# victorramirez952/tomography_3d_reconstructor

Hardware: NVIDIA B200
Metric: Gvoxels/s mask-stack->mesh+volume (higher is better)
Workload: dtype u8 -> bit-packed u32 (topology), f64 field taps -> f32 vertices

## Files before the change

tomography_3d_reconstructor_b200/csrc/t3d_common.cuh:

```cuda
#pragma once
#include <cuda_runtime.h>
#include <stdint.h>
#include <stdio.h>

int t3d_num_sms(void);
#define T3D_NUM_SMS (t3d_num_sms())
bool t3d_first_use_on_device(int slot);
enum { T3D_ONCE_FILL_HOLES_ATTR = 0, T3D_ONCE_MC_LUTS = 1, T3D_ONCE_SORT_ATTR = 2, T3D_ONCE_MORPH4_ATTR = 3, T3D_ONCE_SLOTS = 8 };

extern "C" void t3d_set_error(const char* fmt, ...);
extern "C" void t3d_count_launches(int n);
int t3d_zero_async(void* p, size_t n, cudaStream_t st);
void t3d_prezero_register(const void* p, size_t n);
void t3d_prezero_clear(void);
void t3d_canonicalize_structured_zero_range(int64_t V, int64_t F, uint32_t cap_z, uint32_t cap_g0, int Zs, int64_t* offset,
                                            int64_t* size);

#define T3D_CHECK_LAUNCH(name)                                                                   \
    do {                                                                                         \
        cudaError_t e__ = cudaGetLastError();                                                    \
        if (e__ != cudaSuccess) {                                                                \
            t3d_set_error("%s: launch failed: %s", name, cudaGetErrorString(e__));               \
            return 1;                                                                            \
        }                                                                                        \
    } while (0)

#define T3D_CUDA(call)                                                                           \
    do {                                                                                         \
        cudaError_t e__ = (call);                                                                \
        if (e__ != cudaSuccess) {                                                                \
            t3d_set_error("%s failed: %s", #call, cudaGetErrorString(e__));                      \
            return 1;                                                                            \
        }                                                                                        \
    } while (0)

static inline int t3d_wpr(int W) { return (((W + 31) >> 5) + 3) & ~3; }
static inline int t3d_wvalid(int W) { return (W + 31) >> 5; }

__device__ __forceinline__ uint32_t lane_id() { return threadIdx.x & 31; }

__device__ __forceinline__ uint32_t valid_mask(int w, int W)
{
    const int rem = W - (w << 5);
    if (rem >= 32) return 0xffffffffu;
    if (rem <= 0) return 0u;
    return (1u << rem) - 1u;
}

template <typename T>
__device__ __forceinline__ T warp_sum(T v)
{
#pragma unroll
    for (int o = 16; o > 0; o >>= 1) v += __shfl_xor_sync(0xffffffffu, v, o);
    return v;
}

__device__ __forceinline__ int warp_min(int v)
{
#pragma unroll
    for (int o = 16; o > 0; o >>= 1) v = min(v, __shfl_xor_sync(0xffffffffu, v, o));
    return v;
}
__device__ __forceinline__ int warp_max(int v)
{
#pragma unroll
    for (int o = 16; o > 0; o >>= 1) v = max(v, __shfl_xor_sync(0xffffffffu, v, o));
    return v;
}

__device__ __forceinline__ uint32_t warp_incl_scan(uint32_t v)
{
    const uint32_t l = lane_id();
#pragma unroll
    for (int o = 1; o < 32; o <<= 1) {
        uint32_t t = __shfl_up_sync(0xffffffffu, v, o);
        if (l >= (uint32_t)o) v += t;
    }
    return v;
}

__device__ __forceinline__ uint4 ld_stream_u4(const void* p)
{
    uint4 r;
    asm volatile("ld.global.nc.L1::no_allocate.v4.u32 {%0,%1,%2,%3}, [%4];"
                 : "=r"(r.x), "=r"(r.y), "=r"(r.z), "=r"(r.w)
                 : "l"(p));
    return r;
}
__device__ __forceinline__ void st_stream_u4(void* p, uint4 v)
{
    asm volatile("st.global.L1::no_allocate.v4.u32 [%0], {%1,%2,%3,%4};" ::"l"(p), "r"(v.x), "r"(v.y),
                 "r"(v.z), "r"(v.w)
                 : "memory");
}

__device__ __forceinline__ uint32_t ge4(uint32_t v, uint32_t thr4)
{
    const uint32_t m = __vcmpgeu4(v, thr4) & 0x80808080u;
    return (m * 0x00204081u) >> 28;
}
__device__ __forceinline__ uint32_t ge16(uint4 v, uint32_t thr4)
{
    return ge4(v.x, thr4) | (ge4(v.y, thr4) << 4) | (ge4(v.z, thr4) << 8) | (ge4(v.w, thr4) << 12);
}
__device__ __forceinline__ uint32_t expand4(uint32_t nib) { return (nib * 0x00204081u) & 0x01010101u; }

__device__ __forceinline__ uint4 and4(uint4 a, uint4 b) { return make_uint4(a.x & b.x, a.y & b.y, a.z & b.z, a.w & b.w); }
__device__ __forceinline__ uint4 or4(uint4 a, uint4 b) { return make_uint4(a.x | b.x, a.y | b.y, a.z | b.z, a.w | b.w); }
__device__ __forceinline__ uint4 splat4(uint32_t v) { return make_uint4(v, v, v, v); }
__device__ __forceinline__ uint32_t popc4(uint4 a) { return __popc(a.x) + __popc(a.y) + __popc(a.z) + __popc(a.w); }
__device__ __forceinline__ uint4 valid_mask4(int w4, int W)
{
    return make_uint4(valid_mask(4 * w4, W), valid_mask(4 * w4 + 1, W), valid_mask(4 * w4 + 2, W), valid_mask(4 * w4 + 3, W));
}
__device__ __forceinline__ uint4 shl1_4(uint4 c, uint32_t l)
{
    return make_uint4(__funnelshift_l(l, c.x, 1), __funnelshift_l(c.x, c.y, 1), __funnelshift_l(c.y, c.z, 1), __funnelshift_l(c.z, c.w, 1));
}
__device__ __forceinline__ uint4 shr1_4(uint4 c, uint32_t r)
{
    return make_uint4(__funnelshift_r(c.x, c.y, 1), __funnelshift_r(c.y, c.z, 1), __funnelshift_r(c.z, c.w, 1), __funnelshift_r(c.w, r, 1));
}

__device__ __forceinline__ int64_t dev_n(int64_t cap, const unsigned long long* p)
{
    if (!p) return cap;
    const unsigned long long v = *p;
    return v < (unsigned long long)cap ? (int64_t)v : cap;
}

int t3d_morph_stage(const uint32_t* in, uint32_t* out, int Z, int H, int W, int z0, int nz, int out_rs, long long out_ps,
                    bool erode, bool ring, int ring_tail, unsigned long long* counts, cudaStream_t st);
bool t3d_morph4_eligible(int Z, int H, int W);
int t3d_morph4_launch(const uint32_t* in, uint32_t* out, int Z, int H, int W, int z0, int nz, int out_rs, long long out_ps, int ring_tail,
                      unsigned long long* counts, cudaStream_t st);
void t3d_canon_faces_ready_event(cudaEvent_t e);
bool t3d_canon_faces_ready_pending();
bool t3d_pack_gap_supported(const void* masks_u8, int Z, int H, int W, int threshold);
int t3d_pack_gap_launch(const void* masks_u8, int Z, int H, int W, int threshold, void* out, unsigned long long* counts,
                        unsigned int* bbox_t, int skip_ends, cudaStream_t st, int z_bias = 0);
int t3d_bbox_t_planes_launch(const uint32_t* bits, int n_planes, int H, int W, int z_bias, unsigned int* bbox_t, cudaStream_t st);
int t3d_close_ends_fixup_launch(const void* masks_u8, int Z, int H, int W, int threshold, const void* filled0, const void* filledT,
                                void* out, unsigned long long* counts, cudaStream_t st);
```

tomography_3d_reconstructor_b200/csrc/t3d_pipeline.cu:

```cuda
#include <stdint.h>

#include <stdlib.h>

#include <nvtx3/nvToolsExt.h>

#include "t3d.h"
#include "t3d_field.cuh"

struct NvtxRange {
    bool open;
    explicit NvtxRange(const char* name) : open(true) { nvtxRangePushA(name); }
    void end() { if (open) { nvtxRangePop(); open = false; } }
    ~NvtxRange() { end(); }
};

enum {
    R_NACTIVE = 0, R_NX = 1, R_NY = 2, R_NZ = 3, R_NT = 4, R_VCANON = 5, R_FCANON = 6, R_UNVERIFIED = 7, R_OVERFLOW = 8,
    R_NAMBIGUOUS = 9, R_NEXACT = 10, R_VOLUME_F64 = 11, R_AREA_F64 = 12, R_BBOX_I32X6 = 13 , R_VRAW = 16, R_NEXC = 17,
    R_NGHOST = 18, R_NLEAD = 19, R_NG0 = 25,
    R_COUNTS = 32
};

#define EXC_CAP (1u << 20)
#define SURF_HALO 3

#define S_XPAD 128

static inline int64_t al(int64_t x) { return (x + 255) & ~(int64_t)255; }

static bool fast_surface(int n_stages, unsigned erode_mask, int pad, int Zx, int H, int W)
{
    return pad == 1 && n_stages == 4 && (erode_mask & 15u) == 9u && Zx >= 2 && H >= 2 && W >= 2;
}

struct Layout {
    int64_t bitsA, bitsB, bitsC, morph, fill, sign, exc, ballots, chunkbase, scan1, aw_idx, aw_cnt, aw_base, scan2, vkeys, verts_raw,
        faces_raw, canon, measure, total;
};

static Layout make_layout(int Zx, int Zl, int H, int W, int pad, uint32_t capNA, uint32_t capV, uint32_t capF, uint32_t capZ,
                          uint32_t capG0, int n_stages, bool own_bitsA, bool fast)
{
    Layout L;
    const int64_t nw = t3d_words_per_row(W), vol = (int64_t)Zx * H * nw * 4;
    const int Zp = Zl + 2 * pad, Hp = H + 2 * pad, Wp = fast ? W + S_XPAD + 1 : W + 2 * pad;
    const int64_t nwp = t3d_words_per_row(Wp), n_chunks = t3d_mc_num_chunks(Zp, Hp, Wp);
    int64_t o = 0;
    L.bitsA = o; o += own_bitsA ? al(vol) : 0;
    L.bitsB = o; o += al(vol);
    L.bitsC = o; o += fast ? 0 : al(vol);
    L.morph = o; o += al(t3d_morph_scratch_bytes(Zx, H, W, n_stages));
    L.fill = o; o += al(t3d_fill_holes_scratch_bytes(2, H, W));
    L.sign = o; o += al((int64_t)Zp * Hp * nwp * 4);
    L.exc = o; o += al((int64_t)EXC_CAP * 8);
    L.ballots = o; o += al(n_chunks * 4);
    L.chunkbase = o; o += al(n_chunks * 4);
    L.scan1 = o; o += al(t3d_scan_workspace_bytes(n_chunks, 1));
    L.aw_idx = o; o += al((int64_t)capNA * 4);
    L.aw_cnt = o; o += al((int64_t)capNA * 16);
    L.aw_base = o; o += al((int64_t)capNA * 16);
    L.scan2 = o; o += al(t3d_scan_workspace_bytes(capNA, 4));
    L.vkeys = o; o += al((int64_t)capV * 8);
    L.verts_raw = o; o += al((int64_t)capV * 12);
    L.faces_raw = o; o += al((int64_t)capF * 12);
    L.canon = o; o += al(capZ ? t3d_canonicalize_structured_workspace_bytes(capV, capF, capZ, capG0, Zp)
                              : t3d_canonicalize_fast_workspace_bytes(capV, capF));
    L.measure = o; o += al(t3d_mesh_measure_workspace_bytes());
    L.total = o;
    return L;
}

extern "C" int64_t t3d_reconstruct_workspace_bytes(int Z, int H, int W, int add_padding, int n_stages, uint32_t cap_active,
                                                   uint32_t cap_verts, uint32_t cap_faces, uint32_t cap_zverts, uint32_t cap_g0)
{
    const int pad = add_padding ? 1 : 0;
    const int64_t a = make_layout(Z, Z, H, W, pad, cap_active, cap_verts, cap_faces, cap_zverts, cap_g0, n_stages, true, false).total;
    const int64_t b = make_layout(Z, Z, H, W, pad, cap_active, cap_verts, cap_faces, cap_zverts, cap_g0, n_stages, true, true).total;
    return a > b ? a : b;
}

extern "C" int64_t t3d_reconstruct_results_len(int Z) { return R_COUNTS + 2 * (int64_t)Z; }

static inline int imin(int a, int b) { return a < b ? a : b; }

extern "C" int64_t t3d_reconstruct_slab_workspace_bytes(int halo_lo, int n_own, int halo_hi, int H, int W, int add_padding,
                                                        int n_stages, uint32_t cap_active, uint32_t cap_verts, uint32_t cap_faces,
                                                        uint32_t cap_zverts, uint32_t cap_g0)
{
    const int Zx = halo_lo + n_own + halo_hi, Zl = imin(SURF_HALO, halo_lo) + n_own + imin(SURF_HALO, halo_hi);
    const int pad = add_padding ? 1 : 0;
    const int64_t a = make_layout(Zx, Zl, H, W, pad, cap_active, cap_verts, cap_faces, cap_zverts, cap_g0, n_stages, false, false).total;
    const int64_t b = make_layout(Zx, Zl, H, W, pad, cap_active, cap_verts, cap_faces, cap_zverts, cap_g0, n_stages, false, true).total;
    return a > b ? a : b;
}

__global__ void k_finalize_sizes(unsigned long long* r, unsigned long long capNA, unsigned long long capV, unsigned long long capF,
                                 int bbox_transformed)
{
    if (bbox_transformed) {
        unsigned int* t = (unsigned int*)(r + R_BBOX_I32X6);
        int* b = (int*)(r + R_BBOX_I32X6);
        for (int k = 0; k < 3; ++k) {
            const unsigned lo = t[2 * k], hi = t[2 * k + 1];
            b[2 * k] = 0x7fffffff - (int)lo;
            b[2 * k + 1] = (int)hi - 1;
        }
    }
    unsigned long long of8 = (r[R_NEXC] > EXC_CAP) ? 8ull : 0ull;
    const unsigned long long v = r[R_NX] + r[R_NY] + r[R_NZ];
    r[R_VRAW] = v;
    unsigned long long of = 0;
    if (r[R_NACTIVE] > capNA) of |= 1;
    if (v > capV) of |= 2;
    if (r[R_NT] > capF) of |= 4;
    r[R_OVERFLOW] = of | of8;
    if (of | of8) {
        for (int k = 0; k < 5; ++k) { r[20 + k] = r[R_NACTIVE + k]; r[R_NACTIVE + k] = 0; }
        r[R_VRAW] = 0;
    }
}

__global__ void k_count_plane_vertices(const float* __restrict__ verts, const unsigned long long* n_dev, float z_ghost, float z_lead,
                                       int want_ghost, int want_lead, unsigned long long* out_ghost, unsigned long long* out_lead)
{
    const int w = threadIdx.x >> 5, lane = threadIdx.x & 31;
    const bool want = w == 0 ? want_ghost != 0 : want_lead != 0;
    unsigned long long* out = w == 0 ? out_ghost : out_lead;
    if (!want) {
        if (lane == 0) *out = 0;
        return;
    }
    const float zq = w == 0 ? z_ghost : z_lead;
    const long long n = (long long)*n_dev;
    long long bound[2];
    for (int upper = 0; upper < 2; ++upper) {
        long long lo = 0, hi = n;
        while (hi - lo > 0) {
            const long long span = hi - lo, step = (span + 31) / 32;
            const long long i = lo + (long long)lane * step;
            bool before = false;
            if (i < hi) {
                const float z = verts[3 * i];
                before = upper ? (z <= zq) : (z < zq);
            }
            const unsigned b = __ballot_sync(0xffffffffu, before);
            const int k = __popc(b);
            if (k == 0) { hi = lo; break; }
            const long long last_before = lo + (long long)(k - 1) * step;
            const long long nlo = last_before + 1;
            const long long nhi = (k < 32 && lo + (long long)k * step < hi) ? lo + (long long)k * step : hi;
            lo = nlo; hi = nhi;
        }
        bound[upper] = lo;
    }
    if (lane == 0) *out = (unsigned long long)(bound[1] - bound[0]);
}

#define N_SIDE_EVENTS 8
struct SideStream {
    cudaStream_t s = nullptr;
    cudaEvent_t e[N_SIDE_EVENTS] = {};
};
static SideStream g_side[64];

static int side_for_current_device(SideStream** out)
{
    int dev = 0;
    T3D_CUDA(cudaGetDevice(&dev));
    SideStream& s = g_side[dev & 63];
    if (!s.s) {
        int prio_lo = 0, prio_hi = 0;
        T3D_CUDA(cudaDeviceGetStreamPriorityRange(&prio_lo, &prio_hi));
        T3D_CUDA(cudaStreamCreateWithPriority(&s.s, cudaStreamNonBlocking, prio_hi));
        for (int k = 0; k < N_SIDE_EVENTS; ++k) T3D_CUDA(cudaEventCreateWithFlags(&s.e[k], cudaEventDisableTiming));
    }
    *out = &s;
    return 0;
}

#define RUN(call) do { if (int rc__ = (call)) return rc__; } while (0)

struct ZeroSet {
    uint4* p[6];
    unsigned long long n16[6];
    int n;
};
__global__ void __launch_bounds__(256) k_zero_ranges(ZeroSet z)
{
    for (int k = 0; k < z.n; ++k)
        for (unsigned long long i = (unsigned long long)blockIdx.x * blockDim.x + threadIdx.x; i < z.n16[k];
             i += (unsigned long long)gridDim.x * blockDim.x)
            z.p[k][i] = make_uint4(0, 0, 0, 0);
}
struct PrezeroGuard {
    PrezeroGuard() { t3d_prezero_clear(); }
    ~PrezeroGuard() { t3d_prezero_clear(); }
    ZeroSet z{};
    void add(void* p, size_t bytes)
    {
        const size_t n16 = bytes / 16;
        if (!n16 || z.n >= 6 || ((uintptr_t)p & 15)) return;
        z.p[z.n] = (uint4*)p; z.n16[z.n] = n16; ++z.n;
        t3d_prezero_register(p, n16 * 16);
    }
    int launch(cudaStream_t st)
    {
        if (!z.n) return 0;
        k_zero_ranges<<<T3D_NUM_SMS * 2, 256, 0, st>>>(z);
        T3D_CHECK_LAUNCH("k_zero_ranges");
        t3d_count_launches(1);
        return 0;
    }
};

struct SlabGeom {
    int hl, n, hh;
    int z_begin, z_end;
    int z_offset;
    int want_ghost, want_lead;
    float z_ghost, z_lead;
};

__global__ void __launch_bounds__(256) k_zero_ring(uint4* __restrict__ S, int Zs, int Hs, int nws4)
{
    const long long plane4 = (long long)Hs * nws4;
    const long long nA = 2 * plane4, nB = (long long)(Zs - 2) * 2 * nws4;
    const uint4 zero = make_uint4(0, 0, 0, 0);
    for (long long i = (long long)blockIdx.x * blockDim.x + threadIdx.x; i < nA + nB; i += (long long)gridDim.x * blockDim.x) {
        if (i < nA) {
            S[i < plane4 ? i : (long long)(Zs - 1) * plane4 + (i - plane4)] = zero;
        } else {
            const long long j = i - nA;
            const long long z = 1 + j / (2 * nws4);
            const int r = (int)(j % (2 * nws4));
            S[z * plane4 + (long long)(r < nws4 ? 0 : Hs - 1) * nws4 + (r % nws4)] = zero;
        }
    }
}

struct StageMarks {
    enum { N = 12 };
    cudaEvent_t ev[N];
    const char* name[N];
    int n = 0;
    bool on = false;
    void begin(cudaStream_t st)
    {
        static const bool want = getenv("T3D_STAGE_EVENTS") != nullptr;
        on = false;
        if (!want) return;
        cudaStreamCaptureStatus cs = cudaStreamCaptureStatusNone;
        if (cudaStreamIsCapturing(st, &cs) != cudaSuccess || cs != cudaStreamCaptureStatusNone) return;
        on = true; n = 0;
    }
    void mark(const char* what, cudaStream_t st)
    {
        if (!on || n >= N) return;
        static thread_local cudaEvent_t pool[N] = {};
        if (!pool[n]) cudaEventCreate(&pool[n]);
        ev[n] = pool[n]; name[n] = what;
        cudaEventRecord(ev[n], st);
        ++n;
    }
    void report(cudaStream_t st)
    {
        if (!on) return;
        cudaStreamSynchronize(st);
        fprintf(stderr, "[t3d stages]");
        for (int i = 1; i < n; ++i) { float ms = 0; cudaEventElapsedTime(&ms, ev[i - 1], ev[i]); fprintf(stderr, " %s %.1f us |", name[i], 1e3f * ms); }
        float tot = 0; if (n > 1) cudaEventElapsedTime(&tot, ev[0], ev[n - 1]);
        fprintf(stderr, " total %.1f us\n", 1e3f * tot);
    }
};

static int reconstruct_core(const uint32_t* grid, const SlabGeom& g, int H, int W, int n_stages, unsigned erode_mask, int pad,
                            const double* weights3_host, const void* cum_f64, const void* adj_f64, int n_cum, double mm_y,
                            double mm_x, int scale_in_f64, uint32_t cap_active, uint32_t cap_verts, uint32_t cap_faces,
                            uint32_t cap_zverts, uint32_t cap_g0, int zkey_bits, void* verts_out_f32, void* faces_out_i64,
                            unsigned long long* R, char* ws, const Layout& L, bool fast, int bbox_state, SideStream* side, cudaStream_t st)
{
    const int Zx = g.hl + g.n + g.hh;
    const int64_t nw = t3d_words_per_row(W), plane_words = (int64_t)H * nw, vol_words = (int64_t)Zx * plane_words;
    const int sl = imin(SURF_HALO, g.hl), sh = imin(SURF_HALO, g.hh), Zl = sl + g.n + sh;
    const int Zp = Zl + 2 * pad, Hp = H + 2 * pad, Wp = fast ? W + S_XPAD + 1 : W + 2 * pad;
    const int64_t n_chunks = t3d_mc_num_chunks(Zp, Hp, Wp);

    NvtxRange r_smooth("t3d:smooth_voxel_data");
    StageMarks marks;
    marks.begin(st);
    marks.mark("start", st);
    (void)t3d_canon_faces_ready_pending();
    T3D_CUDA(cudaEventRecord(side->e[2], st));
    T3D_CUDA(cudaStreamWaitEvent(side->s, side->e[2], 0));
    if (bbox_state == 0)
        RUN(t3d_volume_stats(grid + (int64_t)g.hl * plane_words, g.n, H, W, nullptr, R + R_BBOX_I32X6, side->s));
    OccView view;
    int x_off = 0;
    if (fast) {
        const int nws = (int)t3d_words_per_row(Wp);
        uint32_t* S = (uint32_t*)(ws + L.sign);
        const long long s_ps = (long long)Hp * nws;
        {
            const long long items = 2 * (long long)Hp * (nws / 4) + (long long)(Zp - 2) * 2 * (nws / 4);
            long long blocks = (items + 255) / 256;
            if (blocks > (long long)T3D_NUM_SMS * 8) blocks = (long long)T3D_NUM_SMS * 8;
            k_zero_ring<<<(unsigned)(blocks < 1 ? 1 : blocks), 256, 0, side->s>>>((uint4*)S, Zp, Hp, nws / 4);
            t3d_count_launches(1);
        }
        T3D_CUDA(cudaEventRecord(side->e[3], side->s));
        uint32_t* tA = (uint32_t*)(ws + L.morph);
        uint32_t* tB = tA + vol_words;
        uint32_t* S_origin = S + s_ps + nws + S_XPAD / 32;
        const int z0 = g.hl - sl;
        const int ring_tail = (nws - (int)nw - S_XPAD / 32) / 4;
        if (t3d_morph4_eligible(Zx, H, W)) {
            RUN(t3d_morph4_launch(grid, S_origin, Zx, H, W, z0, Zl, nws, s_ps, ring_tail, R + R_COUNTS + Zx + z0, st));
        } else {
            RUN(t3d_morph_stage(grid, tA, Zx, H, W, 0, Zx, (int)nw, plane_words, true, false, 0, nullptr, st));
            RUN(t3d_morph_stage(tA, tB, Zx, H, W, 0, Zx, (int)nw, plane_words, false, false, 0, nullptr, st));
            RUN(t3d_morph_stage(tB, tA, Zx, H, W, 0, Zx, (int)nw, plane_words, false, false, 0, nullptr, st));
            RUN(t3d_morph_stage(tA, S_origin, Zx, H, W, z0, Zl, nws, s_ps, true, true, ring_tail, R + R_COUNTS + Zx + z0, st));
        }
        view = t3d_make_view_strided(S_origin, Zl, H, W, nws, s_ps, 1, 1, weights3_host);
        x_off = S_XPAD - 1;
        T3D_CUDA(cudaStreamWaitEvent(st, side->e[3], 0));
    } else {
        T3D_CUDA(cudaEventRecord(side->e[3], side->s));
        uint32_t* bitsC = (uint32_t*)(ws + L.bitsC);
        const uint32_t* smoothed = grid;
        if (n_stages > 0) {
            RUN(t3d_morph(grid, bitsC, Zx, H, W, n_stages, erode_mask, R + R_COUNTS + Zx, ws + L.morph, st));
            smoothed = bitsC;
        } else {
            T3D_CUDA(cudaMemcpyAsync(R + R_COUNTS + Zx, R + R_COUNTS, sizeof(unsigned long long) * Zx, cudaMemcpyDeviceToDevice, st));
        }
        const uint32_t* surf = smoothed + (int64_t)(g.hl - sl) * plane_words;
        RUN(t3d_field_sign_lean(surf, Zl, H, W, pad, weights3_host, ws + L.sign, R + R_NEXACT, ws + L.exc, EXC_CAP, R + R_NEXC, st));
        view = t3d_make_view(surf, Zl, H, W, pad, 1, weights3_host);
    }

    r_smooth.end();
    marks.mark("smooth", st);
    NvtxRange r_mc("t3d:extract_manifold_surface");
    RUN(t3d_mc_flags(ws + L.sign, Zp, Hp, Wp, g.z_begin, g.z_end, ws + L.ballots, st));
    marks.mark("flags", st);
    RUN(t3d_exclusive_scan_u32_dev(ws + L.ballots, ws + L.chunkbase, n_chunks, n_chunks, 1, 0, 1, nullptr, R + R_NACTIVE,
                                   ws + L.scan1, st));
    RUN(t3d_mc_words_view_dev(view, x_off, ws + L.sign, Zp, Hp, Wp, g.z_begin, g.z_end, ws + L.ballots, ws + L.chunkbase, cap_active,
                              R + R_NACTIVE, ws + L.aw_idx, ws + L.aw_cnt, R + R_NAMBIGUOUS, st));
    RUN(t3d_exclusive_scan_u32_dev(ws + L.aw_cnt, ws + L.aw_base, cap_active, cap_active, 4, 0, 0, R + R_NACTIVE, R + R_NX,
                                   ws + L.scan2, st));
    k_finalize_sizes<<<1, 1, 0, st>>>(R, cap_active, cap_verts, cap_faces, bbox_state == 2 ? 1 : 0);
    t3d_count_launches(1);
    marks.mark("scan+words+scan", st);
    RUN(t3d_mc_emit_view_dev(view, x_off, ws + L.sign, Zp, Hp, Wp, g.z_begin, g.z_end, ws + L.ballots, ws + L.chunkbase, ws + L.aw_idx,
                             ws + L.aw_base, cap_active, R + R_NACTIVE, cap_verts, cap_faces, ws + L.vkeys, ws + L.faces_raw, 1, st));
    marks.mark("keys", st);
    RUN(t3d_mc_vertices_view_dev(view, x_off, ws + L.vkeys, R + R_NACTIVE, cap_verts, 1, g.z_offset, cum_f64, adj_f64, n_cum, mm_y, mm_x,
                                 scale_in_f64, 7, ws + L.verts_raw, st));
    r_mc.end();
    marks.mark("vertices", st);
    NvtxRange r_canon("t3d:ensure_manifold_mesh+measures");
    T3D_CUDA(cudaEventRecord(side->e[4], st));
    T3D_CUDA(cudaStreamWaitEvent(side->s, side->e[4], 0));
    RUN(t3d_mc_emit_view_dev(view, x_off, ws + L.sign, Zp, Hp, Wp, g.z_begin, g.z_end, ws + L.ballots, ws + L.chunkbase, ws + L.aw_idx,
                             ws + L.aw_base, cap_active, R + R_NACTIVE, cap_verts, cap_faces, ws + L.vkeys, ws + L.faces_raw, 2, side->s));
    T3D_CUDA(cudaEventRecord(side->e[6], side->s));
    RUN(t3d_mesh_measure_dev(ws + L.verts_raw, ws + L.faces_raw, cap_faces, R + R_NT, 0, R + R_VOLUME_F64, ws + L.measure, side->s));
    T3D_CUDA(cudaEventRecord(side->e[5], side->s));
    t3d_canon_faces_ready_event(side->e[6]);
    if (cap_zverts)
        RUN(t3d_mesh_canonicalize_structured_dev(ws + L.verts_raw, ws + L.vkeys, cap_verts, R + R_NACTIVE, R + R_VRAW, Zp, Hp, Wp,
                                                 ws + L.chunkbase, ws + L.aw_base, cap_active, g.z_offset, 1, cum_f64, adj_f64, n_cum,
                                                 zkey_bits, cap_zverts, cap_g0, ws + L.faces_raw, cap_faces, R + R_NT, verts_out_f32,
                                                 faces_out_i64, nullptr, R + R_VCANON, R + R_NG0, ws + L.canon, 3, st));
    else
        RUN(t3d_mesh_canonicalize_fast_dev(ws + L.verts_raw, cap_verts, R + R_VRAW, ws + L.faces_raw, cap_faces, R + R_NT,
                                           verts_out_f32, faces_out_i64, nullptr, R + R_VCANON, ws + L.canon, st));
    if (t3d_canon_faces_ready_pending()) T3D_CUDA(cudaStreamWaitEvent(st, side->e[6], 0));
    if (g.want_ghost || g.want_lead)
        k_count_plane_vertices<<<1, 64, 0, st>>>((const float*)verts_out_f32, R + R_VCANON, g.z_ghost, g.z_lead, g.want_ghost,
                                                 g.want_lead, R + R_NGHOST, R + R_NLEAD);
    if (g.want_ghost || g.want_lead) t3d_count_launches(1);
    marks.mark("canonicalize", st);
    T3D_CUDA(cudaStreamWaitEvent(st, side->e[5], 0));
    marks.mark("wait measures", st);
    marks.report(st);
    return 0;
}

extern "C" int t3d_reconstruct(const void* masks_u8, int Z, int H, int W, int threshold, int close_ends, int n_stages,
                               unsigned erode_mask, int add_padding, const double* weights3_host, const void* cum_f64,
                               const void* adj_f64, int n_cum, double mm_per_pixel_y, double mm_per_pixel_x, int scale_in_f64,
                               uint32_t cap_active, uint32_t cap_verts, uint32_t cap_faces, uint32_t cap_zverts, uint32_t cap_g0,
                               int zkey_bits, void* verts_out_f32, void* faces_out_i64, void* results_u64, void* workspace,
                               void* stream)
{
    if (Z <= 0 || H <= 0 || W <= 0) { t3d_set_error("t3d_reconstruct: empty volume"); return 2; }
    if (cap_active == 0 || cap_verts == 0 || cap_faces == 0) { t3d_set_error("t3d_reconstruct: zero capacity"); return 2; }
    cudaStream_t st = (cudaStream_t)stream;
    const int pad = add_padding ? 1 : 0;
    const bool fast = fast_surface(n_stages, erode_mask, pad, Z, H, W);
    const Layout L = make_layout(Z, Z, H, W, pad, cap_active, cap_verts, cap_faces, cap_zverts, cap_g0, n_stages, true, fast);
    char* ws = (char*)workspace;
    unsigned long long* R = (unsigned long long*)results_u64;
    const int64_t nw = t3d_words_per_row(W), plane_words = (int64_t)H * nw, plane_bytes = (int64_t)H * W;
    uint32_t* bitsA = (uint32_t*)(ws + L.bitsA);
    uint32_t* bitsB = (uint32_t*)(ws + L.bitsB);
    const uint8_t* m = (const uint8_t*)masks_u8;
    SideStream* side;
    RUN(side_for_current_device(&side));
    PrezeroGuard zg;
    {
        const int Zp = Z + 2 * pad, Hp = H + 2 * pad, Wp = fast ? W + S_XPAD + 1 : W + 2 * pad;
        const int64_t n_chunks = t3d_mc_num_chunks(Zp, Hp, Wp);
        zg.add(R, sizeof(unsigned long long) * (R_COUNTS + 2 * (size_t)Z));
        zg.add(ws + L.ballots, (size_t)al(n_chunks * 4));
        zg.add(ws + L.scan1, (size_t)al(t3d_scan_workspace_bytes(n_chunks, 1)));
        zg.add(ws + L.scan2, (size_t)al(t3d_scan_workspace_bytes(cap_active, 4)));
        if (cap_zverts) {
            int64_t off = 0, size = 0;
            t3d_canonicalize_structured_zero_range(cap_verts, cap_faces, cap_zverts, cap_g0, Zp, &off, &size);
            zg.add(ws + L.canon + off, (size_t)size);
        }
        RUN(zg.launch(st));
    }

    int bbox_state = 0;
    NvtxRange r_create("t3d:create_voxel_data");
    if (close_ends && t3d_pack_gap_supported(m, Z, H, W, threshold)) {
        uint32_t* f0 = bitsA;
        uint32_t* fT = bitsA + plane_words;
        RUN(t3d_pack_masks(m, 1, H, W, threshold, f0, st));
        RUN(t3d_pack_masks(m + (int64_t)(Z - 1) * plane_bytes, 1, H, W, threshold, fT, st));
        T3D_CUDA(cudaEventRecord(side->e[0], st));
        T3D_CUDA(cudaStreamWaitEvent(side->s, side->e[0], 0));
        RUN(t3d_fill_holes_2d(f0, 2, plane_words, H, W, ws + L.fill, side->s));
        T3D_CUDA(cudaEventRecord(side->e[1], side->s));
        RUN(t3d_pack_gap_launch(m, Z, H, W, threshold, bitsB, R + R_COUNTS, (unsigned int*)(R + R_BBOX_I32X6), 1, st));
        T3D_CUDA(cudaStreamWaitEvent(st, side->e[1], 0));
        RUN(t3d_close_ends_fixup_launch(m, Z, H, W, threshold, f0, fT, bitsB, R + R_COUNTS, st));
        bbox_state = 2;
    } else if (close_ends && Z >= 3) {
        RUN(t3d_pack_masks(m, 1, H, W, threshold, bitsA, st));
        RUN(t3d_pack_masks(m + (int64_t)(Z - 1) * plane_bytes, 1, H, W, threshold, bitsA + (int64_t)(Z - 1) * plane_words, st));
        T3D_CUDA(cudaEventRecord(side->e[0], st));
        T3D_CUDA(cudaStreamWaitEvent(side->s, side->e[0], 0));
        RUN(t3d_fill_holes_2d(bitsA, 2, (int64_t)(Z - 1) * plane_words, H, W, ws + L.fill, side->s));
        T3D_CUDA(cudaEventRecord(side->e[1], side->s));
        RUN(t3d_pack_masks(m + plane_bytes, Z - 2, H, W, threshold, bitsA + plane_words, st));
        T3D_CUDA(cudaStreamWaitEvent(st, side->e[1], 0));
        RUN(t3d_gap_fill(bitsA, bitsB, nullptr, nullptr, Z, H, W, R + R_COUNTS, st));
    } else if (close_ends) {
        RUN(t3d_pack_masks(m, Z, H, W, threshold, bitsA, st));
        RUN(t3d_fill_holes_2d(bitsA, 1, 0, H, W, ws + L.fill, st));
        if (Z > 1) RUN(t3d_fill_holes_2d(bitsA + (int64_t)(Z - 1) * plane_words, 1, 0, H, W, ws + L.fill, st));
        RUN(t3d_gap_fill(bitsA, bitsB, nullptr, nullptr, Z, H, W, R + R_COUNTS, st));
    } else {
        RUN(t3d_pack_masks(m, Z, H, W, threshold, bitsB, st));
        RUN(t3d_volume_stats(bitsB, Z, H, W, R + R_COUNTS, nullptr, st));
    }
    r_create.end();
    SlabGeom g = {0, Z, 0, 0, -1, 0, 0, 0, 0.f, 0.f};
    RUN(reconstruct_core(bitsB, g, H, W, n_stages, erode_mask, pad, weights3_host, cum_f64, adj_f64, n_cum, mm_per_pixel_y,
                         mm_per_pixel_x, scale_in_f64, cap_active, cap_verts, cap_faces, cap_zverts, cap_g0, zkey_bits, verts_out_f32,
                         faces_out_i64, R, ws, L, fast, bbox_state, side, st));
    T3D_CHECK_LAUNCH("t3d_reconstruct");
    t3d_count_launches(1);
    return 0;
}

int t3d_mc_normals_view_dev(const OccView& view, int x_off, const void* vkeys_u64, const void* sizes_u64, uint32_t cap_verts, int unpad_shift,
                            int z_offset, const void* adj_f64, int n_cum, double mm_per_pixel_y, double mm_per_pixel_x,
                            const void* newid_u32, const void* perm_u32, const void* dup_u64, void* winner_u32, void* normals_f32,
                            void* stream);

extern "C" int t3d_reconstruct_normals(int Z, int H, int W, int n_stages, unsigned erode_mask, int add_padding, const double* weights3_host,
                                       const void* adj_f64, int n_cum, double mm_per_pixel_y, double mm_per_pixel_x, uint32_t cap_active,
                                       uint32_t cap_verts, uint32_t cap_faces, uint32_t cap_zverts, uint32_t cap_g0, const void* results_u64,
                                       void* workspace, void* normals_out_f32, void* stream)
{
    if (Z <= 0 || H <= 0 || W <= 0) { t3d_set_error("t3d_reconstruct_normals: empty volume"); return 2; }
    if (cap_active == 0 || cap_verts == 0 || cap_faces == 0) { t3d_set_error("t3d_reconstruct_normals: zero capacity"); return 2; }
    const int pad = add_padding ? 1 : 0;
    const bool fast = fast_surface(n_stages, erode_mask, pad, Z, H, W);
    const Layout L = make_layout(Z, Z, H, W, pad, cap_active, cap_verts, cap_faces, cap_zverts, cap_g0, n_stages, true, fast);
    char* ws = (char*)workspace;
    const unsigned long long* R = (const unsigned long long*)results_u64;
    const int Zp = Z + 2 * pad, Hp = H + 2 * pad, Wp = fast ? W + S_XPAD + 1 : W + 2 * pad;
    OccView view;
    int x_off = 0;
    if (fast) {
        const int nws = (int)t3d_words_per_row(Wp);
        const long long s_ps = (long long)Hp * nws;
        const uint32_t* S_origin = (const uint32_t*)(ws + L.sign) + s_ps + nws + S_XPAD / 32;
        view = t3d_make_view_strided(S_origin, Z, H, W, nws, s_ps, 1, 1, weights3_host);
        x_off = S_XPAD - 1;
    } else {
        const void* smoothed = n_stages > 0 ? ws + L.bitsC : ws + L.bitsB;
        view = t3d_make_view(smoothed, Z, H, W, pad, 1, weights3_host);
    }
    int64_t off[4];
    RUN(t3d_canonical_map_offsets(cap_zverts ? 2 : 1, cap_verts, cap_faces, cap_zverts, cap_g0, Zp, off));
    char* canon = ws + L.canon;
    (void)Hp;
    return t3d_mc_normals_view_dev(view, x_off, ws + L.vkeys, R + R_NACTIVE, cap_verts, 1, 0, adj_f64, n_cum, mm_per_pixel_y,
                                   mm_per_pixel_x, canon + off[0], canon + off[1], canon + off[3], canon + off[2], normals_out_f32,
                                   stream);
}

__global__ void k_merge_pre_stats(unsigned long long* __restrict__ r, const unsigned long long* __restrict__ pre, int Zx, int za, int zb)
{
    const int z = blockIdx.x * blockDim.x + threadIdx.x;
    if (z >= za && z < zb) r[R_COUNTS + z] = pre[z];
    if (z < 6) atomicMax((unsigned int*)(r + R_BBOX_I32X6) + z, ((const unsigned int*)(pre + Zx))[z]);
}

#define SLAB_EDGE 4
#define SLAB_RAW 8

extern "C" int t3d_slab_pack_gap_ok(const void* masks_u8, int n_own, int H, int W, int threshold)
{
    if (n_own < 2 * SLAB_RAW || H <= 0 || W <= 0) return 0;
    const uint8_t* sub = (const uint8_t*)masks_u8 + (int64_t)(SLAB_EDGE - 2) * H * W;
    return t3d_pack_gap_supported(sub, n_own - 2 * SLAB_EDGE + 4, H, W, threshold) ? 1 : 0;
}

extern "C" int t3d_slab_pack(const void* masks_u8, int n_own, int H, int W, int threshold, int halo_lo, int halo_hi, int fill_first,
                             int fill_last, void* ext_bits, void* fill_scratch, void* pre_grid_bits, void* pre_stats_u64, void* stream)
{
    if (n_own <= 0 || H <= 0 || W <= 0 || halo_lo < 0) { t3d_set_error("t3d_slab_pack: bad slab"); return 2; }
    cudaStream_t st = (cudaStream_t)stream;
    const int64_t nw = t3d_words_per_row(W), plane_words = (int64_t)H * nw, plane_bytes = (int64_t)H * W;
    const uint8_t* m = (const uint8_t*)masks_u8;
    uint32_t* own = (uint32_t*)ext_bits + (int64_t)halo_lo * plane_words;
    const bool pre = pre_grid_bits != nullptr;
    if (pre) {
        if (!pre_stats_u64 || !t3d_slab_pack_gap_ok(masks_u8, n_own, H, W, threshold)) {
            t3d_set_error("t3d_slab_pack: pre-filled mode needs pre_stats_u64 and a slab t3d_slab_pack_gap_ok accepts");
            return 2;
        }
        const int Zx = halo_lo + n_own + halo_hi, a0 = SLAB_EDGE - 2, zsub = n_own - 2 * SLAB_EDGE + 4;
        unsigned long long* ps = (unsigned long long*)pre_stats_u64;
        T3D_CUDA(cudaMemsetAsync(ps, 0, sizeof(unsigned long long) * ((size_t)Zx + 3), st));
        RUN(t3d_pack_gap_launch(m + (int64_t)a0 * plane_bytes, zsub, H, W, threshold,
                                (uint32_t*)pre_grid_bits + (int64_t)(halo_lo + a0) * plane_words, ps + halo_lo + a0,
                                (unsigned int*)(ps + Zx), 1, st, a0));
    }
    if (fill_last && n_own == 1 && fill_first) fill_last = 0;
    if (!fill_first && !fill_last) {
        if (!pre) return t3d_pack_masks(m, n_own, H, W, threshold, own, st);
        RUN(t3d_pack_masks(m, SLAB_RAW, H, W, threshold, own, st));
        return t3d_pack_masks(m + (int64_t)(n_own - SLAB_RAW) * plane_bytes, SLAB_RAW, H, W, threshold, own + (int64_t)(n_own - SLAB_RAW) * plane_words, st);
    }
    SideStream* side;
    RUN(side_for_current_device(&side));
    const int lo = fill_first ? 1 : 0, hi = fill_last ? n_own - 1 : n_own;
    if (fill_first) RUN(t3d_pack_masks(m, 1, H, W, threshold, own, st));
    if (fill_last) RUN(t3d_pack_masks(m + (int64_t)(n_own - 1) * plane_bytes, 1, H, W, threshold, own + (int64_t)(n_own - 1) * plane_words, st));
    T3D_CUDA(cudaEventRecord(side->e[0], st));
    T3D_CUDA(cudaStreamWaitEvent(side->s, side->e[0], 0));
    char* scratch = (char*)fill_scratch;
    if (fill_first && fill_last) {
        RUN(t3d_fill_holes_2d(own, 2, (int64_t)(n_own - 1) * plane_words, H, W, scratch, side->s));
    } else {
        RUN(t3d_fill_holes_2d(fill_first ? own : own + (int64_t)(n_own - 1) * plane_words, 1, 0, H, W, scratch, side->s));
    }
    T3D_CUDA(cudaEventRecord(side->e[1], side->s));
    if (pre) {
        RUN(t3d_pack_masks(m + (int64_t)lo * plane_bytes, SLAB_RAW - lo, H, W, threshold, own + (int64_t)lo * plane_words, st));
        const int b0 = n_own - SLAB_RAW;
        RUN(t3d_pack_masks(m + (int64_t)b0 * plane_bytes, hi - b0, H, W, threshold, own + (int64_t)b0 * plane_words, st));
    } else if (hi > lo) RUN(t3d_pack_masks(m + (int64_t)lo * plane_bytes, hi - lo, H, W, threshold, own + (int64_t)lo * plane_words, st));
    const int halo = halo_lo > halo_hi ? halo_lo : halo_hi;
    if (n_own <= halo) T3D_CUDA(cudaStreamWaitEvent(st, side->e[1], 0));
    return 0;
}

extern "C" int t3d_reconstruct_slab(const void* ext_bits, int halo_lo, int n_own, int halo_hi, int H, int W, int n_stages,
                                    unsigned erode_mask, int add_padding, int z_begin, int z_end, int z_offset, int want_ghost,
                                    float z_ghost, int want_lead, float z_lead, int join_fill, const double* weights3_host, const void* cum_f64,
                                    const void* adj_f64, int n_cum, double mm_per_pixel_y, double mm_per_pixel_x, int scale_in_f64,
                                    uint32_t cap_active, uint32_t cap_verts, uint32_t cap_faces, uint32_t cap_zverts, uint32_t cap_g0,
                                    int zkey_bits, void* verts_out_f32, void* faces_out_i64, void* results_u64, void* workspace,
                                    void* pre_grid_bits, const void* pre_stats_u64, void* stream)
{
    if (n_own <= 0 || H <= 0 || W <= 0 || halo_lo < 0 || halo_hi < 0) { t3d_set_error("t3d_reconstruct_slab: bad slab"); return 2; }
    if (pre_grid_bits && (!pre_stats_u64 || n_own < 2 * SLAB_RAW)) { t3d_set_error("t3d_reconstruct_slab: bad pre-filled slab"); return 2; }
    if (cap_active == 0 || cap_verts == 0 || cap_faces == 0) { t3d_set_error("t3d_reconstruct_slab: zero capacity"); return 2; }
    cudaStream_t st = (cudaStream_t)stream;
    const int pad = add_padding ? 1 : 0, Zx = halo_lo + n_own + halo_hi;
    const int Zl = imin(SURF_HALO, halo_lo) + n_own + imin(SURF_HALO, halo_hi);
    const bool fast = fast_surface(n_stages, erode_mask, pad, Zx, H, W);
    const Layout L = make_layout(Zx, Zl, H, W, pad, cap_active, cap_verts, cap_faces, cap_zverts, cap_g0, n_stages, false, fast);
    char* ws = (char*)workspace;
    unsigned long long* R = (unsigned long long*)results_u64;
    SideStream* side;
    RUN(side_for_current_device(&side));
    PrezeroGuard zg;
    {
        const int Zp = Zl + 2 * pad, Hp = H + 2 * pad, Wp = fast ? W + S_XPAD + 1 : W + 2 * pad;
        const int64_t n_chunks = t3d_mc_num_chunks(Zp, Hp, Wp);
        zg.add(R, sizeof(unsigned long long) * (R_COUNTS + 2 * (size_t)Zx));
        zg.add(ws + L.ballots, (size_t)al(n_chunks * 4));
        zg.add(ws + L.scan1, (size_t)al(t3d_scan_workspace_bytes(n_chunks, 1)));
        zg.add(ws + L.scan2, (size_t)al(t3d_scan_workspace_bytes(cap_active, 4)));
        if (cap_zverts) {
            int64_t off = 0, size = 0;
            t3d_canonicalize_structured_zero_range(cap_verts, cap_faces, cap_zverts, cap_g0, Zp, &off, &size);
            zg.add(ws + L.canon + off, (size_t)size);
        }
        RUN(zg.launch(st));
    }
    if (join_fill) T3D_CUDA(cudaStreamWaitEvent(st, side->e[1], 0));
    SlabGeom g = {halo_lo, n_own, halo_hi, z_begin, z_end, z_offset, want_ghost, want_lead, z_ghost, z_lead};
    const uint32_t* grid = (const uint32_t*)(ws + L.bitsB);
    int bbox_state = 0;
    if (pre_grid_bits) {
        const int64_t pw = (int64_t)H * t3d_words_per_row(W);
        const uint32_t* ext = (const uint32_t*)ext_bits;
        uint32_t* pg = (uint32_t*)pre_grid_bits;
        const int zl = halo_lo + SLAB_EDGE, p0 = halo_lo + n_own - SLAB_EDGE;
        RUN(t3d_gap_fill(ext, pg, nullptr, ext + (int64_t)zl * pw, zl, H, W, R + R_COUNTS, st));
        RUN(t3d_gap_fill(ext + (int64_t)p0 * pw, pg + (int64_t)p0 * pw, ext + (int64_t)(p0 - 1) * pw, nullptr, Zx - p0, H, W, R + R_COUNTS + p0, st));
        k_merge_pre_stats<<<(Zx + 255) / 256, 256, 0, st>>>(R, (const unsigned long long*)pre_stats_u64, Zx, zl, p0);
        t3d_count_launches(1);
        unsigned int* bb = (unsigned int*)(R + R_BBOX_I32X6);
        RUN(t3d_bbox_t_planes_launch(pg + (int64_t)halo_lo * pw, SLAB_EDGE, H, W, 0, bb, st));
        RUN(t3d_bbox_t_planes_launch(pg + (int64_t)p0 * pw, SLAB_EDGE, H, W, n_own - SLAB_EDGE, bb, st));
        grid = pg;
        bbox_state = 2;
    } else {
        RUN(t3d_gap_fill(ext_bits, ws + L.bitsB, nullptr, nullptr, Zx, H, W, R + R_COUNTS, st));
    }
    RUN(reconstruct_core(grid, g, H, W, n_stages, erode_mask, pad, weights3_host, cum_f64, adj_f64, n_cum,
                         mm_per_pixel_y, mm_per_pixel_x, scale_in_f64, cap_active, cap_verts, cap_faces, cap_zverts, cap_g0, zkey_bits,
                         verts_out_f32, faces_out_i64, R, ws, L, fast, bbox_state, side, st));
    T3D_CHECK_LAUNCH("t3d_reconstruct_slab");
    t3d_count_launches(1);
    return 0;
}

__global__ void k_add_vertex_base(long long* __restrict__ faces, const unsigned long long* __restrict__ gathered, int64_t stride, int rank,
                                  int64_t cap3)
{
    long long base = 0;
    for (int r = 0; r < rank; ++r) base += (long long)(gathered[r * stride + R_VCANON] - gathered[r * stride + R_NGHOST]);
    const int64_t n3 = 3 * (int64_t)gathered[rank * stride + R_FCANON];
    const int64_t n = n3 < cap3 ? n3 : cap3;
    if (base == 0) return;
    for (int64_t i = (int64_t)blockIdx.x * blockDim.x + threadIdx.x; i < n; i += (int64_t)gridDim.x * blockDim.x) faces[i] += base;
}

extern "C" int t3d_slab_stitch_faces(void* faces_i64, int64_t cap_faces, const void* gathered_results_u64, int64_t stride_u64,
                                     int rank, void* stream)
{
    if (rank < 0 || cap_faces < 0) { t3d_set_error("t3d_slab_stitch_faces: bad arguments"); return 2; }
    if (rank == 0 || cap_faces == 0) return 0;
    k_add_vertex_base<<<T3D_NUM_SMS * 8, 256, 0, (cudaStream_t)stream>>>((long long*)faces_i64, (const unsigned long long*)gathered_results_u64,
                                                               stride_u64, rank, 3 * cap_faces);
    T3D_CHECK_LAUNCH("t3d_slab_stitch_faces");
    t3d_count_launches(1);
    return 0;
}
```

tomography_3d_reconstructor_b200/csrc/t3d_surface.cu:

```cuda
#include <stdlib.h>

#include <cub/device/device_radix_sort.cuh>

#include "t3d_field.cuh"

#define FY 8

__device__ __noinline__ uint32_t exact_sign_bits(const OccView* v, int zp, int yp, int wp, uint32_t need, uint32_t s)
{
    while (need) {
        const int b = __ffs(need) - 1;
        need &= need - 1;
        if (field_value(*v, zp, yp, (wp << 5) + b) > 0.5f) s |= 1u << b; else s &= ~(1u << b);
    }
    return s;
}

__device__ __forceinline__ uint4 prow4(const OccView& v, int zp, int yp, int wp4, uint32_t& left, uint32_t& right)
{
    const int z = zp - v.pad, y = yp - v.pad;
    if (z < 0 || z >= v.Z || y < 0 || y >= v.H) { left = right = 0u; return make_uint4(0, 0, 0, 0); }
    const uint32_t* row = v.bits + (z * v.ps + (long long)y * v.rs);
    const int w0 = 4 * wp4;
    const uint4 o = (w0 < v.nw) ? *reinterpret_cast<const uint4*>(row + w0) : make_uint4(0, 0, 0, 0);
    const uint32_t om1 = (w0 >= 1 && w0 - 1 < v.nw) ? row[w0 - 1] : 0u;
    const uint32_t o4 = (w0 + 4 < v.nw) ? row[w0 + 4] : 0u;
    if (!v.pad) { left = om1; right = o4; return o; }
    const uint32_t om2 = (w0 >= 2 && w0 - 2 < v.nw) ? row[w0 - 2] : 0u;
    left = __funnelshift_l(om2, om1, 1);
    right = __funnelshift_l(o.w, o4, 1);
    return make_uint4(__funnelshift_l(om1, o.x, 1), __funnelshift_l(o.x, o.y, 1), __funnelshift_l(o.y, o.z, 1),
                      __funnelshift_l(o.z, o.w, 1));
}

template <bool LEAN>
__global__ void __launch_bounds__(256, LEAN ? 4 : 2) k_field_sign(OccView v, uint32_t* __restrict__ sign, int nwp, int lanes_x,
                                                    int pz_per_block, int fy, unsigned long long* __restrict__ n_exact,
                                                    unsigned long long* __restrict__ exc, unsigned long long exc_cap,
                                                    unsigned long long* __restrict__ exc_count)
{
    __shared__ OccView sv;
    if (!LEAN) {
        if (threadIdx.x == 0) sv = v;
        __syncthreads();
    }
    const int lx = threadIdx.x % lanes_x, pz = threadIdx.x / lanes_x;
    const int nwp4 = nwp >> 2;
    const int wp4 = blockIdx.x * lanes_x + lx, zp = blockIdx.z * pz_per_block + pz, y0 = blockIdx.y * fy;
    if (pz >= pz_per_block || wp4 >= nwp4 || zp >= v.Zp) return;
    const uint4 vm = valid_mask4(wp4, v.Wp);
    const int zm_i = reflect_idx(zp - 1, v.Zp), zq_i = reflect_idx(zp + 1, v.Zp);
    const int last = v.Wp - 1, last_w = last >> 5;
    const uint32_t last_bit = 1u << (last & 31);
    uint32_t l0, r0, lc, rc, ln, rn;
    uint4 prev = prow4(v, zp, reflect_idx(y0 - 1, v.Hp), wp4, l0, r0);
    uint4 cur = prow4(v, zp, y0, wp4, lc, rc);
    const int y1 = min(v.Hp, y0 + fy);
    for (int yp = y0; yp < y1; ++yp) {
        const uint4 next = prow4(v, zp, reflect_idx(yp + 1, v.Hp), wp4, ln, rn);
        uint32_t d0, d1;
        const uint4 zm = prow4(v, zm_i, yp, wp4, d0, d1), zq = prow4(v, zq_i, yp, wp4, d0, d1);
        uint4 xm = shl1_4(cur, lc), xq = shr1_4(cur, rc);
        if (wp4 == 0) xm.x = (xm.x & ~1u) | (cur.x & 1u);
        if ((last_w >> 2) == wp4) {
            const int j = last_w & 3;
            if (j == 0) xq.x = (xq.x & ~last_bit) | (cur.x & last_bit);
            else if (j == 1) xq.y = (xq.y & ~last_bit) | (cur.y & last_bit);
            else if (j == 2) xq.z = (xq.z & ~last_bit) | (cur.z & last_bit);
            else xq.w = (xq.w & ~last_bit) | (cur.w & last_bit);
        }
        const uint4 any1 = or4(or4(or4(zm, zq), or4(prev, next)), or4(xm, xq));
        const uint4 all1 = and4(and4(and4(zm, zq), and4(prev, next)), and4(xm, xq));
        uint4 s = and4(cur, any1);
        uint4 need;
        need.x = ((cur.x & ~any1.x) | (~cur.x & all1.x)) & vm.x;
        need.y = ((cur.y & ~any1.y) | (~cur.y & all1.y)) & vm.y;
        need.z = ((cur.z & ~any1.z) | (~cur.z & all1.z)) & vm.z;
        need.w = ((cur.w & ~any1.w) | (~cur.w & all1.w)) & vm.w;
        if (need.x | need.y | need.z | need.w) {
            atomicAdd(n_exact, (unsigned long long)popc4(need));
            if (LEAN) {
                const unsigned long long flat = ((unsigned long long)zp * v.Hp + yp) * nwp + 4 * wp4;
                const uint32_t nd[4] = {need.x, need.y, need.z, need.w};
#pragma unroll
                for (int j = 0; j < 4; ++j) {
                    if (nd[j]) {
                        const unsigned long long k = atomicAdd(exc_count, 1ull);
                        if (k < exc_cap) exc[k] = ((flat + j) << 32) | nd[j];
                    }
                }
            } else {
                if (need.x) s.x = exact_sign_bits(&sv, zp, yp, 4 * wp4, need.x, s.x);
                if (need.y) s.y = exact_sign_bits(&sv, zp, yp, 4 * wp4 + 1, need.y, s.y);
                if (need.z) s.z = exact_sign_bits(&sv, zp, yp, 4 * wp4 + 2, need.z, s.z);
                if (need.w) s.w = exact_sign_bits(&sv, zp, yp, 4 * wp4 + 3, need.w, s.w);
            }
        }
        *reinterpret_cast<uint4*>(sign + ((int64_t)zp * v.Hp + yp) * nwp + 4 * wp4) = and4(s, vm);
        prev = cur;
        cur = next; lc = ln; rc = rn;
    }
}

__global__ void __launch_bounds__(128) k_field_sign_fix(OccView v, uint32_t* __restrict__ sign, int nwp,
                                                        const unsigned long long* __restrict__ exc, unsigned long long exc_cap,
                                                        const unsigned long long* __restrict__ exc_count)
{
    const unsigned long long n = min(*exc_count, exc_cap);
    for (unsigned long long i = (unsigned long long)blockIdx.x * blockDim.x + threadIdx.x; i < n; i += (unsigned long long)gridDim.x * blockDim.x) {
        const unsigned long long e = exc[i];
        const unsigned long long flat = e >> 32;
        uint32_t need = (uint32_t)e;
        const int wp = (int)(flat % nwp);
        const unsigned long long row = flat / nwp;
        const int yp = (int)(row % v.Hp), zp = (int)(row / v.Hp);
        uint32_t s = sign[flat];
        while (need) {
            const int b = __ffs(need) - 1;
            need &= need - 1;
            if (field_value(v, zp, yp, (wp << 5) + b) > 0.5f) s |= 1u << b; else s &= ~(1u << b);
        }
        sign[flat] = s;
    }
}

#define SC_THREADS 256
#define SC_ITEMS 8
#define SC_TILE (SC_THREADS * SC_ITEMS)
#define SC_FLAG_A (1ull << 62)
#define SC_FLAG_P (2ull << 62)
#define SC_VALUE_MASK ((1ull << 62) - 1)

template <typename OutT>
__global__ void __launch_bounds__(SC_THREADS) k_scan_lookback(const uint32_t* __restrict__ in, OutT* __restrict__ out, int64_t n_cap,
                                                              int64_t stride, unsigned long long* __restrict__ desc, int n_tiles,
                                                              unsigned int* __restrict__ tickets, int popc_in,
                                                              const unsigned long long* __restrict__ n_dev,
                                                              unsigned long long* __restrict__ totals)
{
    const int64_t n = dev_n(n_cap, n_dev);
    const uint32_t* a = in + (int64_t)blockIdx.y * stride;
    OutT* o = out + (int64_t)blockIdx.y * stride;
    volatile unsigned long long* d = desc + (int64_t)blockIdx.y * n_tiles;
    __shared__ int s_tile;
    __shared__ uint32_t sh[SC_THREADS / 32];
    __shared__ unsigned long long s_prefix;
    if (threadIdx.x == 0) s_tile = (int)atomicAdd(tickets + blockIdx.y, 1u);
    __syncthreads();
    const int tile = s_tile;
    const int64_t need = (n + SC_TILE - 1) / SC_TILE;
    n_tiles = (int)(need < 1 ? 1 : (need < n_tiles ? need : n_tiles));
    if (tile >= n_tiles) return;
    const int64_t base = (int64_t)tile * SC_TILE + (int64_t)threadIdx.x * SC_ITEMS;
    uint32_t v[SC_ITEMS];
    uint32_t sum = 0;
#pragma unroll
    for (int k = 0; k < SC_ITEMS; ++k) {
        v[k] = (base + k < n) ? (popc_in ? (uint32_t)__popc(a[base + k]) : a[base + k]) : 0u;
        sum += v[k];
    }
    const uint32_t incl = warp_incl_scan(sum);
    if (lane_id() == 31) sh[threadIdx.x >> 5] = incl;
    __syncthreads();
    uint32_t woff = 0, agg = 0;
#pragma unroll
    for (int k = 0; k < SC_THREADS / 32; ++k) {
        if (k < (int)(threadIdx.x >> 5)) woff += sh[k];
        agg += sh[k];
    }
    if (threadIdx.x < 32) {
        unsigned long long prefix = 0;
        if (tile == 0) {
            if (threadIdx.x == 0) { d[0] = SC_FLAG_P | (unsigned long long)agg; }
        } else {
            if (threadIdx.x == 0) { d[tile] = SC_FLAG_A | (unsigned long long)agg; }
            int idx = tile - 1 - (int)threadIdx.x;
            while (true) {
                unsigned long long w = (idx >= 0) ? d[idx] : SC_FLAG_P;
                while (__any_sync(0xffffffffu, (w >> 62) == 0)) {
                    if ((w >> 62) == 0) w = (idx >= 0) ? d[idx] : SC_FLAG_P;
                }
                const uint32_t is_p = __ballot_sync(0xffffffffu, (w >> 62) == 2);
                const int first_p = is_p ? (__ffs(is_p) - 1) : 32;
                unsigned long long val = ((int)threadIdx.x <= first_p) ? (w & SC_VALUE_MASK) : 0ull;
#pragma unroll
                for (int off = 16; off > 0; off >>= 1) val += __shfl_xor_sync(0xffffffffu, val, off);
                prefix += val;
                if (is_p) break;
                idx -= 32;
            }
            if (threadIdx.x == 0) { d[tile] = SC_FLAG_P | ((prefix + agg) & SC_VALUE_MASK); }
        }
        if (threadIdx.x == 0) {
            s_prefix = prefix;
            if (tile == n_tiles - 1) totals[blockIdx.y] = prefix + agg;
        }
    }
    __syncthreads();
    unsigned long long run = s_prefix + woff + (incl - sum);
#pragma unroll
    for (int k = 0; k < SC_ITEMS; ++k) {
        if (base + k < n) o[base + k] = (OutT)run;
        run += v[k];
    }
}

extern "C" int64_t t3d_scan_workspace_bytes(int64_t n, int n_arrays)
{
    const int64_t nb = (n + SC_THREADS * 4 - 1) / (SC_THREADS * 4);
    return (nb * n_arrays + 16) * 8 + 256;
}

extern "C" int t3d_exclusive_scan_u32_dev(const void* in, void* out, int64_t n_cap, int64_t stride, int n_arrays, int out_is_u64,
                                          int popcount_input, const void* n_dev_u64, void* totals_u64, void* workspace, void* stream)
{
    cudaStream_t st = (cudaStream_t)stream;
    if (n_cap <= 0 || n_arrays <= 0) {
        if (n_arrays > 0) T3D_CUDA(cudaMemsetAsync(totals_u64, 0, 8 * n_arrays, st));
        return 0;
    }
    if (n_arrays > 16) { t3d_set_error("t3d_exclusive_scan_u32_dev: at most 16 arrays per call"); return 2; }
    const int64_t nb = (n_cap + SC_TILE - 1) / SC_TILE;
    if (nb > 0x7fffffff) { t3d_set_error("t3d_exclusive_scan_u32_dev: too many elements"); return 2; }
    const size_t desc_bytes = (size_t)nb * n_arrays * 8;
    if (t3d_zero_async(workspace, desc_bytes + 64, st)) return 1;
    unsigned long long* desc = (unsigned long long*)workspace;
    unsigned int* tickets = (unsigned int*)((char*)workspace + desc_bytes);
    const unsigned long long* nd = (const unsigned long long*)n_dev_u64;
    dim3 grid((unsigned)nb, n_arrays);
    if (out_is_u64)
        k_scan_lookback<unsigned long long><<<grid, SC_THREADS, 0, st>>>((const uint32_t*)in, (unsigned long long*)out, n_cap, stride, desc,
                                                                         (int)nb, tickets, popcount_input, nd,
                                                                         (unsigned long long*)totals_u64);
    else
        k_scan_lookback<uint32_t><<<grid, SC_THREADS, 0, st>>>((const uint32_t*)in, (uint32_t*)out, n_cap, stride, desc, (int)nb, tickets,
                                                               popcount_input, nd, (unsigned long long*)totals_u64);
    T3D_CHECK_LAUNCH("t3d_exclusive_scan_u32_dev");
    t3d_count_launches(1);
    return 0;
}

extern "C" int t3d_field_sign(const void* occ_bits, int Z, int H, int W, int pad, const double* weights3, void* sign_bits,
                              void* n_exact_u64, void* stream)
{
    if (Z <= 0 || H <= 0 || W <= 0) { t3d_set_error("t3d_field_sign: empty volume"); return 2; }
    cudaStream_t st = (cudaStream_t)stream;
    const OccView v = t3d_make_view(occ_bits, Z, H, W, pad, 1, weights3);
    const int nwp = t3d_wpr(v.Wp);
    T3D_CUDA(cudaMemsetAsync(n_exact_u64, 0, 8, st));
    const int nwp4 = nwp / 4, lanes_x = nwp4 < 256 ? nwp4 : 256, pzb = 256 / lanes_x;
    dim3 grid((nwp4 + lanes_x - 1) / lanes_x, (v.Hp + FY - 1) / FY, (v.Zp + pzb - 1) / pzb);
    k_field_sign<false><<<grid, 256, 0, st>>>(v, (uint32_t*)sign_bits, nwp, lanes_x, pzb, FY, (unsigned long long*)n_exact_u64, nullptr, 0,
                                              nullptr);
    T3D_CHECK_LAUNCH("t3d_field_sign");
    t3d_count_launches(1);
    return 0;
}

extern "C" int t3d_field_sign_lean(const void* occ_bits, int Z, int H, int W, int pad, const double* weights3, void* sign_bits,
                                   void* n_exact_u64, void* exc_list_u64, uint32_t exc_cap, void* exc_count_u64, void* stream)
{
    if (Z <= 0 || H <= 0 || W <= 0) { t3d_set_error("t3d_field_sign_lean: empty volume"); return 2; }
    cudaStream_t st = (cudaStream_t)stream;
    const OccView v = t3d_make_view(occ_bits, Z, H, W, pad, 1, weights3);
    const int nwp = t3d_wpr(v.Wp);
    if (t3d_zero_async(n_exact_u64, 8, st) || t3d_zero_async(exc_count_u64, 8, st)) return 1;
    const int nwp4 = nwp / 4, lanes_x = nwp4 < 256 ? nwp4 : 256, pzb = 256 / lanes_x;
    dim3 grid((nwp4 + lanes_x - 1) / lanes_x, (v.Hp + FY - 1) / FY, (v.Zp + pzb - 1) / pzb);
    k_field_sign<true><<<grid, 256, 0, st>>>(v, (uint32_t*)sign_bits, nwp, lanes_x, pzb, FY, (unsigned long long*)n_exact_u64,
                                             (unsigned long long*)exc_list_u64, exc_cap, (unsigned long long*)exc_count_u64);
    k_field_sign_fix<<<T3D_NUM_SMS, 128, 0, st>>>(v, (uint32_t*)sign_bits, nwp, (const unsigned long long*)exc_list_u64, exc_cap,
                                                  (const unsigned long long*)exc_count_u64);
    T3D_CHECK_LAUNCH("t3d_field_sign_lean");
    t3d_count_launches(2);
    return 0;
}

__global__ void __launch_bounds__(256) k_field_dense(OccView v, float* __restrict__ out)
{
    const int64_t i = (int64_t)blockIdx.x * blockDim.x + threadIdx.x;
    const int64_t total = (int64_t)v.Zp * v.Hp * v.Wp;
    if (i >= total) return;
    const int x = (int)(i % v.Wp);
    const int64_t r = i / v.Wp;
    out[i] = field_value(v, (int)(r / v.Hp), (int)(r % v.Hp), x);
}

extern "C" int t3d_field_dense(const void* occ_bits, int Z, int H, int W, int pad, int gaussian, const double* weights3,
                               void* out_f32, void* stream)
{
    if (Z <= 0 || H <= 0 || W <= 0) { t3d_set_error("t3d_field_dense: empty volume"); return 2; }
    const OccView v = t3d_make_view(occ_bits, Z, H, W, pad, gaussian, weights3);
    const int64_t total = (int64_t)v.Zp * v.Hp * v.Wp;
    k_field_dense<<<(unsigned)((total + 255) / 256), 256, 0, (cudaStream_t)stream>>>(v, (float*)out_f32);
    T3D_CHECK_LAUNCH("t3d_field_dense");
    t3d_count_launches(1);
    return 0;
}

__global__ void __launch_bounds__(256) k_cube_cases(const uint32_t* __restrict__ sign, int Zs, int Hs, int Ws, int nws,
                                                    uint8_t* __restrict__ out)
{
    const int64_t i = (int64_t)blockIdx.x * blockDim.x + threadIdx.x;
    const int64_t total = (int64_t)(Zs - 1) * (Hs - 1) * (Ws - 1);
    if (i >= total) return;
    const int x = (int)(i % (Ws - 1));
    const int64_t r = i / (Ws - 1);
    const int y = (int)(r % (Hs - 1)), z = (int)(r / (Hs - 1));
    auto sb = [&](int zz, int yy, int xx) -> int {
        return (int)((sign[((int64_t)zz * Hs + yy) * nws + (xx >> 5)] >> (xx & 31)) & 1u);
    };
    out[i] = (uint8_t)(sb(z, y, x) | (sb(z, y, x + 1) << 1) | (sb(z, y + 1, x + 1) << 2) | (sb(z, y + 1, x) << 3) |
                       (sb(z + 1, y, x) << 4) | (sb(z + 1, y, x + 1) << 5) | (sb(z + 1, y + 1, x + 1) << 6) |
                       (sb(z + 1, y + 1, x) << 7));
}

extern "C" int t3d_cube_cases(const void* sign_bits, int Zs, int Hs, int Ws, void* out_u8, void* stream)
{
    if (Zs < 2 || Hs < 2 || Ws < 2) { t3d_set_error("t3d_cube_cases: volume smaller than 2x2x2"); return 2; }
    const int64_t total = (int64_t)(Zs - 1) * (Hs - 1) * (Ws - 1);
    k_cube_cases<<<(unsigned)((total + 255) / 256), 256, 0, (cudaStream_t)stream>>>((const uint32_t*)sign_bits, Zs, Hs, Ws,
                                                                                  t3d_wpr(Ws), (uint8_t*)out_u8);
    T3D_CHECK_LAUNCH("t3d_cube_cases");
    t3d_count_launches(1);
    return 0;
}

__device__ __forceinline__ uint32_t float_key(float f)
{
    uint32_t u = __float_as_uint(f);
    if (u == 0x80000000u) u = 0u;
    return (u & 0x80000000u) ? ~u : (u | 0x80000000u);
}

__global__ void __launch_bounds__(256) k_make_keys(const float* __restrict__ verts, int64_t V, int col, const uint32_t* __restrict__ perm,
                                                   uint32_t* __restrict__ keys, uint32_t* __restrict__ iota)
{
    const int64_t i = (int64_t)blockIdx.x * blockDim.x + threadIdx.x;
    if (i >= V) return;
    const uint32_t src = perm ? perm[i] : (uint32_t)i;
    keys[i] = float_key(verts[3 * (int64_t)src + col]);
    if (iota) iota[i] = (uint32_t)i;
}

__global__ void __launch_bounds__(256) k_unique_heads(const float* __restrict__ verts, const uint32_t* __restrict__ perm, int64_t V,
                                                      uint32_t* __restrict__ head)
{
    const int64_t i = (int64_t)blockIdx.x * blockDim.x + threadIdx.x;
    if (i >= V) return;
    uint32_t h = 1;
    if (i > 0) {
        const float* a = verts + 3 * (int64_t)perm[i];
        const float* b = verts + 3 * (int64_t)perm[i - 1];
        h = (float_key(a[0]) != float_key(b[0]) || float_key(a[1]) != float_key(b[1]) || float_key(a[2]) != float_key(b[2])) ? 1u : 0u;
    }
    head[i] = h;
}

__global__ void __launch_bounds__(256) k_scatter_unique(const float* __restrict__ verts, const uint32_t* __restrict__ perm,
                                                        const uint32_t* __restrict__ head, const uint32_t* __restrict__ pos,
                                                        int64_t V_cap, float* __restrict__ out_verts, uint32_t* __restrict__ newid,
                                                        const unsigned long long* __restrict__ V_dev = nullptr)
{
    const int64_t i = (int64_t)blockIdx.x * blockDim.x + threadIdx.x;
    if (i >= dev_n(V_cap, V_dev)) return;
    const uint32_t u = pos[i] + head[i] - 1u;
    const uint32_t src = perm[i];
    newid[src] = u;
    if (head[i]) {
        const float* a = verts + 3 * (int64_t)src;
        float* o = out_verts + 3 * (int64_t)u;
        o[0] = a[0]; o[1] = a[1]; o[2] = a[2];
    }
}

__global__ void __launch_bounds__(256) k_face_valid(const int32_t* __restrict__ faces, int64_t F_cap, const uint32_t* __restrict__ newid,
                                                    uint32_t* __restrict__ valid, const unsigned long long* __restrict__ F_dev = nullptr)
{
    const int64_t i = (int64_t)blockIdx.x * blockDim.x + threadIdx.x;
    if (i >= dev_n(F_cap, F_dev)) return;
    const uint32_t a = newid[faces[3 * i]], b = newid[faces[3 * i + 1]], c = newid[faces[3 * i + 2]];
    valid[i] = (a != b && b != c && a != c) ? 1u : 0u;
}

__global__ void __launch_bounds__(256) k_face_compact(const int32_t* __restrict__ faces, int64_t F_cap, const uint32_t* __restrict__ newid,
                                                      const uint32_t* __restrict__ valid, const uint32_t* __restrict__ pos,
                                                      long long* __restrict__ out64, int32_t* __restrict__ out32,
                                                      const unsigned long long* __restrict__ F_dev = nullptr)
{
    const int64_t F = dev_n(F_cap, F_dev);
    for (int64_t i = (int64_t)blockIdx.x * blockDim.x + threadIdx.x; i < F; i += (int64_t)gridDim.x * blockDim.x) {
        if (!valid[i]) continue;
        const uint32_t a = newid[faces[3 * i]], b = newid[faces[3 * i + 1]], c = newid[faces[3 * i + 2]];
        const int64_t o = 3 * (int64_t)pos[i];
        if (out64) { out64[o] = a; out64[o + 1] = b; out64[o + 2] = c; }
        if (out32) { out32[o] = (int32_t)a; out32[o + 1] = (int32_t)b; out32[o + 2] = (int32_t)c; }
    }
}

__global__ void __launch_bounds__(256) k_face_remap(const int32_t* __restrict__ faces, int64_t F_cap, const uint32_t* __restrict__ newid,
                                                    uint32_t* __restrict__ valid, long long* __restrict__ out64, int32_t* __restrict__ out32,
                                                    unsigned long long* __restrict__ n_invalid, const unsigned long long* __restrict__ F_dev)
{
    const int64_t i = (int64_t)blockIdx.x * blockDim.x + threadIdx.x;
    const int64_t F = dev_n(F_cap, F_dev);
    bool bad = false;
    if (i < F) {
        const uint32_t a = newid[faces[3 * i]], b = newid[faces[3 * i + 1]], c = newid[faces[3 * i + 2]];
        bad = !(a != b && b != c && a != c);
        valid[i] = bad ? 0u : 1u;
        if (out64) { out64[3 * i] = a; out64[3 * i + 1] = b; out64[3 * i + 2] = c; }
        if (out32) { out32[3 * i] = (int32_t)a; out32[3 * i + 1] = (int32_t)b; out32[3 * i + 2] = (int32_t)c; }
    }
    const uint32_t nb = __popc(__ballot_sync(0xffffffffu, bad));
    if (lane_id() == 0 && nb) atomicAdd(n_invalid, (unsigned long long)nb);
}

__global__ void k_face_plan(const unsigned long long* __restrict__ n_invalid, int64_t F_cap, const unsigned long long* __restrict__ F_dev,
                            unsigned long long* __restrict__ n_to_compact, unsigned long long* __restrict__ f_out)
{
    const unsigned long long F = (unsigned long long)dev_n(F_cap, F_dev);
    *n_to_compact = (*n_invalid) ? F : 0ull;
    *f_out = F - *n_invalid;
}

static size_t sort_temp_bytes(int64_t V)
{
    size_t bytes = 0;
    cub::DeviceRadixSort::SortPairs(nullptr, bytes, (const uint32_t*)nullptr, (uint32_t*)nullptr, (const uint32_t*)nullptr,
                                    (uint32_t*)nullptr, (int)V);
    return bytes;
}

static inline int64_t align256(int64_t x) { return (x + 255) & ~(int64_t)255; }

extern "C" int64_t t3d_canonicalize_workspace_bytes(int64_t V, int64_t F)
{
    const int64_t n = V > F ? V : F;
    int64_t b = 0;
    b += 4 * align256(4 * V);
    b += 2 * align256(4 * n);
    b += align256(4 * V);
    b += align256((int64_t)sort_temp_bytes(V > 0 ? V : 1));
    b += align256(t3d_scan_workspace_bytes(n, 1));
    b += 256;
    return b;
}

extern "C" int t3d_mesh_canonicalize(const void* verts_in, int64_t V, const void* faces_in, int64_t F, void* verts_out,
                                     void* faces_out_i64, void* faces_out_i32, void* counts_u64, void* workspace, void* stream)
{
    cudaStream_t st = (cudaStream_t)stream;
    if (V <= 0 || V > 0x7fffffff || F < 0) { t3d_set_error("t3d_mesh_canonicalize: bad sizes"); return 2; }
    const int64_t n = V > F ? V : F;
    char* ws = (char*)workspace;
    uint32_t* keys_a = (uint32_t*)ws; ws += align256(4 * V);
    uint32_t* keys_b = (uint32_t*)ws; ws += align256(4 * V);
    uint32_t* perm_a = (uint32_t*)ws; ws += align256(4 * V);
    uint32_t* perm_b = (uint32_t*)ws; ws += align256(4 * V);
    uint32_t* flags = (uint32_t*)ws; ws += align256(4 * n);
    uint32_t* pos = (uint32_t*)ws; ws += align256(4 * n);
    uint32_t* newid = (uint32_t*)ws; ws += align256(4 * V);
    size_t temp_bytes = sort_temp_bytes(V);
    void* temp = ws; ws += align256((int64_t)temp_bytes);
    void* scan_ws = ws; ws += align256(t3d_scan_workspace_bytes(n, 1));
    unsigned long long* totals = (unsigned long long*)ws;
    unsigned long long* counts = (unsigned long long*)counts_u64;
    const unsigned gv = (unsigned)((V + 255) / 256);
    const float* vin = (const float*)verts_in;

    uint32_t *pin = nullptr, *pout = perm_a, *pspare = perm_b;
    for (int pass = 0; pass < 3; ++pass) {
        const int col = 2 - pass;
        k_make_keys<<<gv, 256, 0, st>>>(vin, V, col, pin, keys_a, pass == 0 ? pspare : nullptr);
        const uint32_t* vals_in = (pass == 0) ? pspare : pin;
        T3D_CUDA(cub::DeviceRadixSort::SortPairs(temp, temp_bytes, (const uint32_t*)keys_a, keys_b, vals_in, pout, (int)V, 0, 32, st));
        uint32_t* old_in = pin;
        pin = pout;
        pout = (pass == 0) ? pspare : old_in;
        if (pass == 0) pspare = nullptr;
    }
    const uint32_t* perm = pin;
    k_unique_heads<<<gv, 256, 0, st>>>(vin, perm, V, flags);
    if (t3d_exclusive_scan_u32_dev(flags, pos, V, V, 1, 0, 0, nullptr, totals, scan_ws, stream)) return 1;
    T3D_CUDA(cudaMemcpyAsync(counts, totals, 8, cudaMemcpyDeviceToDevice, st));
    k_scatter_unique<<<gv, 256, 0, st>>>(vin, perm, flags, pos, V, (float*)verts_out, newid);
    if (F > 0) {
        const unsigned gf = (unsigned)((F + 255) / 256);
        k_face_valid<<<gf, 256, 0, st>>>((const int32_t*)faces_in, F, newid, flags);
        if (t3d_exclusive_scan_u32_dev(flags, pos, F, F, 1, 0, 0, nullptr, totals, scan_ws, stream)) return 1;
        T3D_CUDA(cudaMemcpyAsync(counts + 1, totals, 8, cudaMemcpyDeviceToDevice, st));
        k_face_compact<<<gf, 256, 0, st>>>((const int32_t*)faces_in, F, newid, flags, pos, (long long*)faces_out_i64,
                                           (int32_t*)faces_out_i32);
    } else {
        T3D_CUDA(cudaMemsetAsync(counts + 1, 0, 8, st));
    }
    T3D_CHECK_LAUNCH("t3d_mesh_canonicalize");
    t3d_count_launches(F > 0 ? 7 : 5);
    return 0;
}

__global__ void __launch_bounds__(256) k_make_keys64(const float* __restrict__ verts, int64_t V_cap, const unsigned long long* __restrict__ V_dev,
                                                     unsigned long long* __restrict__ keys, uint32_t* __restrict__ iota)
{
    const int64_t i = (int64_t)blockIdx.x * blockDim.x + threadIdx.x;
    if (i >= V_cap) return;
    keys[i] = (i < dev_n(V_cap, V_dev)) ? (((unsigned long long)float_key(verts[3 * i]) << 32) | float_key(verts[3 * i + 1]))
                                        : 0xffffffffffffffffull;
    iota[i] = (uint32_t)i;
}

__global__ void __launch_bounds__(256) k_heads_checked(const float* __restrict__ verts, const uint32_t* __restrict__ perm, int64_t V_cap,
                                                       const unsigned long long* __restrict__ V_dev, uint32_t* __restrict__ head,
                                                       unsigned long long* __restrict__ bad)
{
    const int64_t i = (int64_t)blockIdx.x * blockDim.x + threadIdx.x;
    if (i >= dev_n(V_cap, V_dev)) return;
    uint32_t h = 1;
    if (i > 0) {
        const float* a = verts + 3 * (int64_t)perm[i];
        const float* b = verts + 3 * (int64_t)perm[i - 1];
        const uint32_t az = float_key(a[0]), ay = float_key(a[1]), ax = float_key(a[2]);
        const uint32_t bz = float_key(b[0]), by = float_key(b[1]), bx = float_key(b[2]);
        h = (az != bz || ay != by || ax != bx) ? 1u : 0u;
        const bool lt = (az < bz) || (az == bz && (ay < by || (ay == by && ax < bx)));
        if (lt) atomicOr(bad, 1ull);
    }
    head[i] = h;
}

static size_t sort64_temp_bytes(int64_t V)
{
    size_t bytes = 0;
    cub::DeviceRadixSort::SortPairs(nullptr, bytes, (const unsigned long long*)nullptr, (unsigned long long*)nullptr,
                                    (const uint32_t*)nullptr, (uint32_t*)nullptr, (int)V);
    return bytes;
}

extern "C" int64_t t3d_canonicalize_fast_workspace_bytes(int64_t V, int64_t F)
{
    const int64_t n = V > F ? V : F;
    int64_t b = 0;
    b += 2 * align256(8 * V);
    b += 2 * align256(4 * V);
    b += 2 * align256(4 * n);
    b += align256(4 * V);
    b += align256((int64_t)sort64_temp_bytes(V > 0 ? V : 1));
    b += align256(t3d_scan_workspace_bytes(n, 1));
    b += 256;
    return b;
}

#define UQ_ITEMS 4
#define UQ_TILE (SC_THREADS * UQ_ITEMS)
__global__ void __launch_bounds__(SC_THREADS) k_unique_fused(const float* __restrict__ verts, const uint32_t* __restrict__ perm, int64_t V_cap,
                                                             const unsigned long long* __restrict__ V_dev, float* __restrict__ out_verts,
                                                             uint32_t* __restrict__ newid, unsigned long long* __restrict__ desc, int n_tiles,
                                                             unsigned int* __restrict__ ticket, unsigned long long* __restrict__ bad,
                                                             unsigned long long* __restrict__ n_unique_out,
                                                             const unsigned long long* __restrict__ skip_unless)
{
    if (skip_unless && *skip_unless == 0) return;
    const int64_t n = dev_n(V_cap, V_dev);
    volatile unsigned long long* d = desc;
    __shared__ int s_tile;
    __shared__ uint32_t s_kz[UQ_TILE + 1], s_ky[UQ_TILE + 1], s_kx[UQ_TILE + 1];
    __shared__ uint32_t s_part[UQ_ITEMS * (SC_THREADS / 32)];
    __shared__ unsigned long long s_prefix;
    if (threadIdx.x == 0) s_tile = (int)atomicAdd(ticket, 1u);
    __syncthreads();
    const int tile = s_tile;
    const int64_t need = (n + UQ_TILE - 1) / UQ_TILE;
    n_tiles = (int)(need < 1 ? 1 : (need < n_tiles ? need : n_tiles));
    if (tile >= n_tiles) return;
    const int64_t base = (int64_t)tile * UQ_TILE;
    const int tid = threadIdx.x, lane = tid & 31, warp = tid >> 5;
    uint32_t src[UQ_ITEMS];
    float vz[UQ_ITEMS], vy[UQ_ITEMS], vx[UQ_ITEMS];
#pragma unroll
    for (int k = 0; k < UQ_ITEMS; ++k) {
        const int e = k * SC_THREADS + tid;
        if (base + e < n) {
            src[k] = perm[base + e];
            const float* a = verts + 3 * (int64_t)src[k];
            vz[k] = a[0]; vy[k] = a[1]; vx[k] = a[2];
            s_kz[e + 1] = float_key(vz[k]); s_ky[e + 1] = float_key(vy[k]); s_kx[e + 1] = float_key(vx[k]);
        }
    }
    if (tid == 0 && base > 0) {
        const float* b = verts + 3 * (int64_t)perm[base - 1];
        s_kz[0] = float_key(b[0]); s_ky[0] = float_key(b[1]); s_kx[0] = float_key(b[2]);
    }
    __syncthreads();
    uint32_t ball[UQ_ITEMS];
    uint32_t myhead = 0;
    bool out_of_order = false;
#pragma unroll
    for (int k = 0; k < UQ_ITEMS; ++k) {
        const int e = k * SC_THREADS + tid;
        bool h = false;
        if (base + e < n) {
            h = true;
            if (base + e > 0) {
                const uint32_t az = s_kz[e + 1], ay = s_ky[e + 1], ax = s_kx[e + 1], pz = s_kz[e], py = s_ky[e], px = s_kx[e];
                h = (az != pz || ay != py || ax != px);
                out_of_order |= (az < pz) || (az == pz && (ay < py || (ay == py && ax < px)));
            }
        }
        ball[k] = __ballot_sync(0xffffffffu, h);
        myhead |= (h ? 1u : 0u) << k;
        if (lane == 0) s_part[k * (SC_THREADS / 32) + warp] = __popc(ball[k]);
    }
    if (out_of_order) atomicOr(bad, 1ull);
    __syncthreads();
    if (tid < 32) {
        constexpr int PER_LANE = UQ_ITEMS * (SC_THREADS / 32) / 32;
        static_assert(PER_LANE >= 1 && PER_LANE * 32 == UQ_ITEMS * (SC_THREADS / 32), "partials must spread evenly over a warp");
        uint32_t pv[PER_LANE], psum = 0;
#pragma unroll
        for (int t = 0; t < PER_LANE; ++t) { pv[t] = s_part[PER_LANE * lane + t]; psum += pv[t]; }
        const uint32_t incl = warp_incl_scan(psum);
        const uint32_t agg = __shfl_sync(0xffffffffu, incl, 31);
        uint32_t runp = incl - psum;
#pragma unroll
        for (int t = 0; t < PER_LANE; ++t) { s_part[PER_LANE * lane + t] = runp; runp += pv[t]; }
        unsigned long long prefix = 0;
        if (tile == 0) {
            if (tid == 0) { d[0] = SC_FLAG_P | (unsigned long long)agg; }
        } else {
            if (tid == 0) { d[tile] = SC_FLAG_A | (unsigned long long)agg; }
            int idx = tile - 1 - tid;
            while (true) {
                unsigned long long w = (idx >= 0) ? d[idx] : SC_FLAG_P;
                while (__any_sync(0xffffffffu, (w >> 62) == 0)) {
                    if ((w >> 62) == 0) w = (idx >= 0) ? d[idx] : SC_FLAG_P;
                }
                const uint32_t is_p = __ballot_sync(0xffffffffu, (w >> 62) == 2);
                const int first_p = is_p ? (__ffs(is_p) - 1) : 32;
                unsigned long long val = (tid <= first_p) ? (w & SC_VALUE_MASK) : 0ull;
#pragma unroll
                for (int off = 16; off > 0; off >>= 1) val += __shfl_xor_sync(0xffffffffu, val, off);
                prefix += val;
                if (is_p) break;
                idx -= 32;
            }
            if (tid == 0) { d[tile] = SC_FLAG_P | ((prefix + agg) & SC_VALUE_MASK); }
        }
        if (tid == 0) {
            s_prefix = prefix;
            if (tile == n_tiles - 1) *n_unique_out = prefix + agg;
        }
    }
    __syncthreads();
    const uint32_t tile_prefix = (uint32_t)s_prefix;
    const uint32_t lt = (1u << lane) - 1u;
#pragma unroll
    for (int k = 0; k < UQ_ITEMS; ++k) {
        const int e = k * SC_THREADS + tid;
        if (base + e < n) {
            const uint32_t h = (myhead >> k) & 1u;
            const uint32_t u = tile_prefix + s_part[k * (SC_THREADS / 32) + warp] + __popc(ball[k] & lt) + h - 1u;
            newid[src[k]] = u;
            if (h) {
                float* o = out_verts + 3 * (int64_t)u;
                o[0] = vz[k]; o[1] = vy[k]; o[2] = vx[k];
            }
        }
    }
}

__global__ void __launch_bounds__(256) k_unique_optimistic(const float* __restrict__ verts, const uint32_t* __restrict__ perm, int64_t V_cap,
                                                           const unsigned long long* __restrict__ V_dev, float* __restrict__ out_verts,
                                                           uint32_t* __restrict__ newid, unsigned long long* __restrict__ bad,
                                                           unsigned long long* __restrict__ n_unique_out, unsigned long long* __restrict__ dup)
{
    const int64_t n = dev_n(V_cap, V_dev);
    const int64_t i = (int64_t)blockIdx.x * blockDim.x + threadIdx.x;
    if (i == 0) *n_unique_out = (unsigned long long)n;
    const bool ok = i < n;
    uint32_t src = 0, kz = 0, ky = 0, kx = 0;
    if (ok) {
        src = perm[i];
        const float* a = verts + 3 * (int64_t)src;
        const float z = a[0], y = a[1], x = a[2];
        float* o = out_verts + 3 * i;
        o[0] = z; o[1] = y; o[2] = x;
        newid[src] = (uint32_t)i;
        kz = float_key(z); ky = float_key(y); kx = float_key(x);
    }
    uint32_t pz = __shfl_up_sync(0xffffffffu, kz, 1), py = __shfl_up_sync(0xffffffffu, ky, 1), px = __shfl_up_sync(0xffffffffu, kx, 1);
    if ((threadIdx.x & 31) == 0 && ok && i > 0) {
        const float* b = verts + 3 * (int64_t)perm[i - 1];
        pz = float_key(b[0]); py = float_key(b[1]); px = float_key(b[2]);
    }
    if (ok && i > 0) {
        if (kz == pz && ky == py && kx == px) atomicOr(dup, 1ull);
        else if ((kz < pz) || (kz == pz && (ky < py || (ky == py && kx < px)))) atomicOr(bad, 1ull);
    }
}

static thread_local cudaEvent_t g_faces_ready = nullptr;
void t3d_canon_faces_ready_event(cudaEvent_t e) { g_faces_ready = e; }
bool t3d_canon_faces_ready_pending() { const bool p = g_faces_ready != nullptr; g_faces_ready = nullptr; return p; }

static int canonical_tail(const float* vin, const uint32_t* perm, int64_t V, const unsigned long long* V_dev, const void* faces_in,
                          int64_t F, const unsigned long long* F_dev, void* verts_out, void* faces_out_i64, void* faces_out_i32,
                          unsigned long long* counts, uint32_t* flags, uint32_t* pos, uint32_t* newid, void* scan_ws,
                          void* scan_ws_faces, unsigned long long* totals, cudaStream_t st)
{
    void* stream = (void*)st;
    {
        const int64_t nb = (V + UQ_TILE - 1) / UQ_TILE;
        const size_t desc_bytes = (size_t)nb * 8;
        if (t3d_zero_async(scan_ws, desc_bytes + 64, st)) return 1;
        unsigned long long* dup = totals + 8;
        if (t3d_zero_async(dup, 8, st)) return 1;
        k_unique_optimistic<<<(unsigned)((V + 255) / 256), 256, 0, st>>>(vin, perm, V, V_dev, (float*)verts_out, newid, counts + 2, counts, dup);
        t3d_count_launches(1);
        k_unique_fused<<<(unsigned)nb, SC_THREADS, 0, st>>>(vin, perm, V, V_dev, (float*)verts_out, newid, (unsigned long long*)scan_ws,
                                                           (int)nb, (unsigned int*)((char*)scan_ws + desc_bytes), counts + 2, counts, dup);
    }
    if (g_faces_ready) {
        T3D_CUDA(cudaStreamWaitEvent(st, g_faces_ready, 0));
        g_faces_ready = nullptr;
    }
    if (F > 0) {
        const unsigned gf = (unsigned)((F + 255) / 256);
        if (t3d_zero_async(totals + 1, 16, st)) return 1;
        k_face_remap<<<gf, 256, 0, st>>>((const int32_t*)faces_in, F, newid, flags, (long long*)faces_out_i64, (int32_t*)faces_out_i32,
                                         totals + 1, F_dev);
        k_face_plan<<<1, 1, 0, st>>>(totals + 1, F, F_dev, totals + 2, counts + 1);
        if (t3d_exclusive_scan_u32_dev(flags, pos, F, F, 1, 0, 0, totals + 2, totals + 3, scan_ws_faces, stream)) return 1;
        const unsigned gc = gf < (unsigned)(T3D_NUM_SMS * 8) ? gf : (unsigned)(T3D_NUM_SMS * 8);
        k_face_compact<<<gc, 256, 0, st>>>((const int32_t*)faces_in, F, newid, flags, pos, (long long*)faces_out_i64,
                                           (int32_t*)faces_out_i32, totals + 2);
    } else {
        T3D_CUDA(cudaMemsetAsync(counts + 1, 0, 8, st));
    }
    return 0;
}

extern "C" int t3d_mesh_canonicalize_fast_dev(const void* verts_in, int64_t V, const void* V_dev_u64, const void* faces_in, int64_t F,
                                              const void* F_dev_u64, void* verts_out, void* faces_out_i64, void* faces_out_i32,
                                              void* counts_u64, void* workspace, void* stream)
{
    cudaStream_t st = (cudaStream_t)stream;
    if (V <= 0 || V > 0x7fffffff || F < 0) { t3d_set_error("t3d_mesh_canonicalize_fast_dev: bad sizes"); return 2; }
    const unsigned long long* V_dev = (const unsigned long long*)V_dev_u64;
    const unsigned long long* F_dev = (const unsigned long long*)F_dev_u64;
    const int64_t n = V > F ? V : F;
    char* ws = (char*)workspace;
    unsigned long long* keys_a = (unsigned long long*)ws; ws += align256(8 * V);
    unsigned long long* keys_b = (unsigned long long*)ws; ws += align256(8 * V);
    uint32_t* iota = (uint32_t*)ws; ws += align256(4 * V);
    uint32_t* perm = (uint32_t*)ws; ws += align256(4 * V);
    uint32_t* flags = (uint32_t*)ws; ws += align256(4 * n);
    uint32_t* pos = (uint32_t*)ws; ws += align256(4 * n);
    uint32_t* newid = (uint32_t*)ws; ws += align256(4 * V);
    size_t temp_bytes = sort64_temp_bytes(V);
    void* temp = ws; ws += align256((int64_t)temp_bytes);
    void* scan_ws = ws; ws += align256(t3d_scan_workspace_bytes(n, 1));
    unsigned long long* totals = (unsigned long long*)ws;
    unsigned long long* counts = (unsigned long long*)counts_u64;
    const unsigned gv = (unsigned)((V + 255) / 256);
    const float* vin = (const float*)verts_in;
    T3D_CUDA(cudaMemsetAsync(counts + 2, 0, 8, st));
    k_make_keys64<<<gv, 256, 0, st>>>(vin, V, V_dev, keys_a, iota);
    T3D_CUDA(cub::DeviceRadixSort::SortPairs(temp, temp_bytes, (const unsigned long long*)keys_a, keys_b, (const uint32_t*)iota, perm,
                                             (int)V, 0, 64, st));
    if (canonical_tail(vin, perm, V, V_dev, faces_in, F, F_dev, verts_out, faces_out_i64, faces_out_i32, counts, flags, pos, newid,
                       scan_ws, scan_ws, totals, st)) return 1;
    T3D_CHECK_LAUNCH("t3d_mesh_canonicalize_fast_dev");
    t3d_count_launches(F > 0 ? 5 : 3);
    return 0;
}

struct CanonS {
    const float* verts;
    const unsigned long long* vkeys;
    const unsigned long long* sizes;
    uint32_t cap_verts, cap_z, cap_g0;
    int Zs, Hs;
    int ncr;
    const uint32_t* chunkbase;
    const uint32_t* aw_base;
    uint32_t stride;
    int g_plane;
    int z_offset; float shift;
    const double* cum; const double* adj; int n_cum;
    int zkey_bits;
    unsigned long long* zkeys;
    uint32_t* zval;
    const uint32_t* zperm;
    unsigned long long* gkeys;
    uint32_t* gval;
    const uint32_t* gperm;
    uint32_t* perm;
    unsigned long long* n_g0_out;
};

template <int AX>
__device__ __forceinline__ uint32_t before_row(const CanonS& c, int64_t row)
{
    const uint32_t na = (uint32_t)c.sizes[0];
    const uint32_t r = row >= (int64_t)c.Zs * c.Hs ? na : c.chunkbase[row * c.ncr];
    return r >= na ? (uint32_t)c.sizes[1 + AX] : c.aw_base[(int64_t)AX * c.stride + r];
}

__device__ __forceinline__ void g0_sizes(const CanonS& c, uint32_t& gX, uint32_t& gY, uint32_t& gZ)
{
    gX = gY = gZ = 0;
    if (c.g_plane < 0) return;
    const int64_t r_plane = (int64_t)min(c.g_plane, c.Zs) * c.Hs, r_next = (int64_t)min(c.g_plane + 1, c.Zs) * c.Hs;
    const uint32_t z_below = before_row<2>(c, r_plane);
    const uint32_t xy_below = before_row<0>(c, r_plane) + before_row<1>(c, r_plane);
    if (z_below == 0 && xy_below == 0) return;
    gX = before_row<0>(c, r_next); gY = before_row<1>(c, r_next); gZ = z_below;
}

__device__ __forceinline__ float plane_z(const CanonS& c, int k)
{
    float fz = __fsub_rn(__double2float_rn((double)(k + c.z_offset)), c.shift);
    if (c.n_cum > 0) {
        if (fz < 0.0f) fz = 0.0f;
        else if (fz >= (float)(c.n_cum - 1)) fz = __double2float_rn(c.cum[c.n_cum - 1]);
        else {
            const float fl = floorf(fz);
            const int lo = (int)fl;
            const float fr = __fsub_rn(fz, fl);
            fz = __double2float_rn(__dadd_rn(c.cum[lo], __dmul_rn((double)fr, c.adj[min(lo, c.n_cum - 2)])));
        }
    }
    return fz;
}

#define ZS_WARPS 16
#define ZS_THREADS (32 * ZS_WARPS)

__device__ __forceinline__ uint32_t canon_zkey(const CanonS& c, uint32_t i, uint32_t nx, uint32_t ny, uint32_t gZ)
{
    if (i < gZ) return 0u;
    const uint32_t raw = nx + ny + i;
    const int k = (int)(c.vkeys[raw] >> 42);
    uint32_t zk = float_key(c.verts[3 * (int64_t)raw]);
    if (c.zkey_bits < 32) {
        const uint32_t base = float_key(plane_z(c, k));
        zk = zk >= base ? zk - base : 0u;
        const uint32_t lim = (1u << c.zkey_bits) - 1u;
        zk = zk > lim ? lim : zk;
    }
    return zk;
}

template <int ZS_U, typename KeyT, typename KeyFn, typename ValFn>
__device__ __forceinline__ void cta_radix_sort_u(uint32_t n, int passes, KeyFn key_of, ValFn value_of, KeyT* keyA, KeyT* keyB, uint32_t* idxA,
                                               uint32_t* idxB, uint32_t* out)
{
    __shared__ uint32_t s_hist[ZS_WARPS][256];
    __shared__ uint32_t s_tot[256];
    __shared__ uint32_t s_carry[8];
    const int tid = threadIdx.x, w = tid >> 5, lane = tid & 31;
    const uint32_t per = (((n + ZS_WARPS - 1) / ZS_WARPS) + 31u) & ~31u;
    const uint32_t ws = min(n, (uint32_t)w * per), we = min(n, ws + per);
    const KeyT* kin = keyA; const uint32_t* iin = idxA;
    KeyT* kout = keyB; uint32_t* iout = idxB;
    for (int p = 0; p < passes; ++p) {
        const int shift = 8 * p;
        const bool first = p == 0, last = p == passes - 1;
        for (int i = tid; i < ZS_WARPS * 256; i += ZS_THREADS) (&s_hist[0][0])[i] = 0;
        __syncthreads();
        for (uint32_t i0 = ws + lane; i0 < we; i0 += 32 * ZS_U) {
            KeyT kk[ZS_U];
#pragma unroll
            for (int u = 0; u < ZS_U; ++u) {
                const uint32_t i = i0 + 32 * u;
                if (i < we) { if (first) { kk[u] = key_of(i); keyA[i] = kk[u]; } else kk[u] = kin[i]; }
            }
#pragma unroll
            for (int u = 0; u < ZS_U; ++u)
                if (i0 + 32 * u < we) atomicAdd(&s_hist[w][(uint32_t)(kk[u] >> shift) & 255u], 1u);
        }
        __syncthreads();
        if (tid < 256) {
            uint32_t t = 0;
            for (int ww = 0; ww < ZS_WARPS; ++ww) t += s_hist[ww][tid];
            s_tot[tid] = t;
        }
        __syncthreads();
        if (tid < 256) {
            const uint32_t v = s_tot[tid];
            const uint32_t incl = warp_incl_scan(v);
            if (lane == 31) s_carry[w] = incl;
            asm volatile("bar.sync 1, 256;" ::: "memory");
            uint32_t carry = 0;
            for (int ww = 0; ww < w; ++ww) carry += s_carry[ww];
            uint32_t run = carry + incl - v;
            for (int ww = 0; ww < ZS_WARPS; ++ww) { const uint32_t h = s_hist[ww][tid]; s_hist[ww][tid] = run; run += h; }
        }
        __syncthreads();
        for (uint32_t c0 = ws; c0 < we; c0 += 32 * ZS_U) {
            KeyT kk[ZS_U];
            uint32_t ii[ZS_U];
#pragma unroll
            for (int u = 0; u < ZS_U; ++u) {
                const uint32_t i = c0 + 32 * u + lane;
                kk[u] = 0; ii[u] = 0;
                if (i < we) {
                    kk[u] = first ? keyA[i] : kin[i];
                    ii[u] = first ? value_of(i) : iin[i];
                }
            }
#pragma unroll
            for (int u = 0; u < ZS_U; ++u) {
                if (c0 + 32 * u >= we) break;
                const uint32_t i = c0 + 32 * u + lane;
                const bool ok = i < we;
                const KeyT key = kk[u];
                const uint32_t idx = ii[u];
                const uint32_t d = ok ? ((uint32_t)(key >> shift) & 255u) : 0xffffffffu;
                const uint32_t peers = __match_any_sync(0xffffffffu, d);
                const uint32_t rank = __popc(peers & ((1u << lane) - 1u));
                uint32_t pos = 0;
                if (ok) pos = s_hist[w][d] + rank;
                __syncwarp();
                if (ok && rank == 0) s_hist[w][d] += __popc(peers);
                __syncwarp();
                if (ok) {
                    if (last) out[pos] = idx;
                    else { kout[pos] = key; iout[pos] = idx; }
                }
            }
        }
        __syncthreads();
        const KeyT* tk = kin; const uint32_t* ti = iin;
        kin = kout; iin = iout;
        kout = (KeyT*)tk; iout = (uint32_t*)ti;
    }
}

template <int ZS_U>
__global__ void __launch_bounds__(ZS_THREADS) k_zsort_layers(CanonS c, uint32_t* __restrict__ keyA, uint32_t* __restrict__ keyB,
                                                            uint32_t* __restrict__ idxA, uint32_t* __restrict__ idxB,
                                                            uint32_t* __restrict__ zperm)
{
    const uint32_t nx = (uint32_t)c.sizes[1], ny = (uint32_t)c.sizes[2], nz = (uint32_t)c.sizes[3];
    if ((unsigned long long)nx + ny + nz > c.cap_verts || nz > c.cap_z) return;
    const int layer = blockIdx.x;
    uint32_t s = before_row<2>(c, (int64_t)layer * c.Hs), e = before_row<2>(c, (int64_t)(layer + 1) * c.Hs);
    if (e > nz) e = nz;
    if (s >= e) return;
    const uint32_t n = e - s;
    uint32_t gX, gY, gZ;
    g0_sizes(c, gX, gY, gZ);
    if (n == 1 || e <= gZ) {
        for (uint32_t i = s + threadIdx.x; i < e; i += ZS_THREADS) zperm[i] = i;
        return;
    }
    cta_radix_sort_u<ZS_U, uint32_t>(n, (c.zkey_bits + 7) / 8, [&](uint32_t i) { return canon_zkey(c, s + i, nx, ny, gZ); },
                                     [&](uint32_t i) { return s + i; }, keyA + s, keyB + s, idxA + s, idxB + s, zperm + s);
}

__global__ void __launch_bounds__(ZS_THREADS) k_gsort(CanonS c, unsigned long long* __restrict__ keyA, unsigned long long* __restrict__ keyB,
                                                     uint32_t* __restrict__ idxA, uint32_t* __restrict__ idxB, uint32_t* __restrict__ gperm)
{
    const uint32_t nx = (uint32_t)c.sizes[1], ny = (uint32_t)c.sizes[2], nz = (uint32_t)c.sizes[3];
    if ((unsigned long long)nx + ny + nz > c.cap_verts) return;
    uint32_t gX, gY, gZ;
    g0_sizes(c, gX, gY, gZ);
    const uint32_t n = gX + gY + gZ;
    if (n == 0 || n > c.cap_g0) return;
    auto raw_of = [&](uint32_t t) -> uint32_t { return t < gX ? t : t < gX + gY ? nx + (t - gX) : nx + ny + (t - gX - gY); };
    if (n == 1) { if (threadIdx.x == 0) gperm[0] = raw_of(0); return; }
    cta_radix_sort_u<1, unsigned long long>(n, 8, [&](uint32_t t) {
        const float* v = c.verts + 3 * (int64_t)raw_of(t);
        return ((unsigned long long)float_key(v[1]) << 32) | float_key(v[2]);
    }, raw_of, keyA, keyB, idxA, idxB, gperm);
}

__global__ void __launch_bounds__(256) k_canon_positions(CanonS c)
{
    __shared__ uint32_t s_g[3];
    const uint32_t i = blockIdx.x * blockDim.x + threadIdx.x;
    const uint32_t nx = (uint32_t)c.sizes[1], ny = (uint32_t)c.sizes[2], nz = (uint32_t)c.sizes[3];
    const unsigned long long V64 = (unsigned long long)nx + ny + nz;
    if (V64 > c.cap_verts) return;
    if (threadIdx.x == 0) g0_sizes(c, s_g[0], s_g[1], s_g[2]);
    __syncthreads();
    if (i >= (uint32_t)V64) return;
    if (nz > c.cap_z) { c.perm[i] = i; return; }
    const uint32_t gX = s_g[0], gY = s_g[1], gZ = s_g[2];
    const uint32_t nG = gX + gY + gZ;
    if (i == 0 && c.n_g0_out) *c.n_g0_out = nG;
    if (i < nG) c.perm[i] = (nG <= c.cap_g0) ? c.gperm[i] : (i < gX ? i : i < gX + gY ? nx + (i - gX) : nx + ny + (i - gX - gY));
    if (i < nx) {
        if (i < gX) return;
        const unsigned long long key = c.vkeys[i];
        const int k = (int)(key >> 42), j = (int)((key >> 22) & 0xfffffu);
        c.perm[i + before_row<1>(c, (int64_t)k * c.Hs + j) + before_row<2>(c, (int64_t)k * c.Hs)] = i;
    } else if (i < nx + ny) {
        const uint32_t iy = i - nx;
        if (iy < gY) return;
        const unsigned long long key = c.vkeys[i];
        const int k = (int)(key >> 42), j = (int)((key >> 22) & 0xfffffu);
        const int64_t row = (int64_t)k * c.Hs + j;
        const uint32_t lo = before_row<1>(c, row), hi = before_row<1>(c, row + 1);
        const uint32_t mine = float_key(c.verts[3 * (int64_t)i + 1]);
        uint32_t r = 0;
        for (uint32_t e = lo; e < hi; ++e) {
            const uint32_t ke = float_key(c.verts[3 * (int64_t)(nx + e) + 1]);
            r += (ke < mine || (ke == mine && e < iy)) ? 1u : 0u;
        }
        c.perm[before_row<0>(c, row + 1) + lo + r + before_row<2>(c, (int64_t)k * c.Hs)] = i;
    } else {
        const uint32_t R = i - nx - ny;
        if (R < gZ) return;
        const uint32_t raw = nx + ny + c.zperm[R];
        const int64_t next_plane = ((int64_t)(c.vkeys[raw] >> 42) + 1) * c.Hs;
        c.perm[before_row<0>(c, next_plane) + before_row<1>(c, next_plane) + R] = raw;
    }
}

extern "C" int64_t t3d_canonicalize_structured_workspace_bytes(int64_t V, int64_t F, uint32_t cap_z, uint32_t cap_g0, int Zs)
{
    const int64_t n = V > F ? V : F;
    int64_t b = 0;
    b += 2 * align256(8 * (int64_t)cap_z) + 2 * align256(4 * (int64_t)cap_z);
    b += 2 * align256(8 * (int64_t)cap_g0) + 2 * align256(4 * (int64_t)cap_g0);
    b += align256(4 * V);
    b += 2 * align256(4 * n);
    b += align256(4 * V);
    b += align256(4 * (int64_t)cap_g0 + 256);
    b += 2 * align256(t3d_scan_workspace_bytes(n, 1)) + 256;
    return b;
}

extern "C" int t3d_canonical_map_offsets(int kind, int64_t V, int64_t F, uint32_t cap_z, uint32_t cap_g0, int Zs, int64_t* out4)
{
    if (V <= 0 || F < 0 || !out4 || kind < 0 || kind > 2) { t3d_set_error("t3d_canonical_map_offsets: bad arguments"); return 2; }
    const int64_t n = V > F ? V : F;
    int64_t o = 0;
    if (kind == 0) {
        out4[1] = 2 * align256(4 * V);
        o = 4 * align256(4 * V);
        out4[2] = o; o += 2 * align256(4 * n);
        out4[0] = o;
        out4[3] = -1;
        return 0;
    }
    if (kind == 1) {
        o = 2 * align256(8 * V) + align256(4 * V);
        out4[1] = o; o += align256(4 * V);
        out4[2] = o; o += 2 * align256(4 * n);
        out4[0] = o; o += align256(4 * V);
        o += align256((int64_t)sort64_temp_bytes(V));
        o += align256(t3d_scan_workspace_bytes(n, 1));
    } else {
        o = 2 * align256(8 * (int64_t)cap_z) + 2 * align256(4 * (int64_t)cap_z) + 2 * align256(8 * (int64_t)cap_g0) +
            2 * align256(4 * (int64_t)cap_g0);
        out4[1] = o; o += align256(4 * V);
        out4[2] = o; o += 2 * align256(4 * n);
        out4[0] = o; o += align256(4 * V);
        o += align256(4 * (int64_t)cap_g0 + 256);
        o += 2 * align256(t3d_scan_workspace_bytes(n, 1));
    }
    out4[3] = o + 8 * 8;
    (void)Zs;
    return 0;
}

void t3d_canonicalize_structured_zero_range(int64_t V, int64_t F, uint32_t cap_z, uint32_t cap_g0, int Zs, int64_t* offset,
                                            int64_t* size)
{
    const int64_t n = V > F ? V : F;
    *size = 2 * align256(t3d_scan_workspace_bytes(n, 1)) + 256;
    *offset = t3d_canonicalize_structured_workspace_bytes(V, F, cap_z, cap_g0, Zs) - *size;
}

extern "C" int t3d_mesh_canonicalize_structured_dev(const void* verts_in, const void* vkeys_u64, int64_t V_cap, const void* sizes_u64,
                                                    const void* V_dev_u64, int Zs, int Hs, int Ws, const void* chunkbase_u32,
                                                    const void* aw_base_u32, uint32_t aw_stride, int z_offset, int unpad_shift,
                                                    const void* cum_f64, const void* adj_f64, int n_cum, int zkey_bits,
                                                    uint32_t cap_z, uint32_t cap_g0, const void* faces_in, int64_t F_cap,
                                                    const void* F_dev_u64, void* verts_out, void* faces_out_i64, void* faces_out_i32,
                                                    void* counts_u64, void* n_g0_u64, void* workspace, int phases, void* stream)
{
    cudaStream_t st = (cudaStream_t)stream;
    if (zkey_bits <= 0 || zkey_bits > 32) zkey_bits = 32;
    if (V_cap <= 0 || V_cap > 0x7fffffff || F_cap < 0 || Zs <= 0 || Hs <= 0 || Ws <= 0 || cap_z == 0 || (phases & 3) == 0) {
        t3d_set_error("t3d_mesh_canonicalize_structured: bad sizes");
        return 2;
    }
    const int64_t V = V_cap, F = F_cap, n = V > F ? V : F;
    char* ws = (char*)workspace;
    CanonS c;
    c.verts = (const float*)verts_in;
    c.vkeys = (const unsigned long long*)vkeys_u64;
    c.sizes = (const unsigned long long*)sizes_u64;
    c.cap_verts = (uint32_t)V; c.cap_z = cap_z; c.cap_g0 = cap_g0;
    c.Zs = Zs; c.Hs = Hs;
    c.ncr = (t3d_wpr(Ws) + 31) >> 5;
    c.chunkbase = (const uint32_t*)chunkbase_u32;
    c.aw_base = (const uint32_t*)aw_base_u32;
    c.stride = aw_stride;
    c.g_plane = (n_cum > 0 && unpad_shift > 0) ? unpad_shift - z_offset : -1;
    c.z_offset = z_offset; c.shift = unpad_shift ? 1.0f : 0.0f;
    c.cum = (const double*)cum_f64; c.adj = (const double*)adj_f64; c.n_cum = n_cum;
    c.zkey_bits = zkey_bits;
    unsigned long long* zkeys_b; uint32_t* zperm; unsigned long long* gkeys_b; uint32_t* gperm;
    c.zkeys = (unsigned long long*)ws; ws += align256(8 * (int64_t)cap_z);
    zkeys_b = (unsigned long long*)ws; ws += align256(8 * (int64_t)cap_z);
    c.zval = (uint32_t*)ws; ws += align256(4 * (int64_t)cap_z);
    zperm = (uint32_t*)ws; ws += align256(4 * (int64_t)cap_z);
    c.gkeys = (unsigned long long*)ws; ws += align256(8 * (int64_t)cap_g0);
    gkeys_b = (unsigned long long*)ws; ws += align256(8 * (int64_t)cap_g0);
    c.gval = (uint32_t*)ws; ws += align256(4 * (int64_t)cap_g0);
    gperm = (uint32_t*)ws; ws += align256(4 * (int64_t)cap_g0);
    c.perm = (uint32_t*)ws; ws += align256(4 * V);
    uint32_t* flags = (uint32_t*)ws; ws += align256(4 * n);
    uint32_t* pos = (uint32_t*)ws; ws += align256(4 * n);
    uint32_t* newid = (uint32_t*)ws; ws += align256(4 * V);
    void* temp = ws; ws += align256(4 * (int64_t)cap_g0 + 256);
    void* scan_ws = ws; ws += align256(t3d_scan_workspace_bytes(n, 1));
    void* scan_ws_f = ws; ws += align256(t3d_scan_workspace_bytes(n, 1));
    unsigned long long* totals = (unsigned long long*)ws;
    unsigned long long* counts = (unsigned long long*)counts_u64;
    c.zperm = zperm; c.gperm = gperm;
    c.n_g0_out = (unsigned long long*)n_g0_u64;
    if (phases & 1) {
        uint32_t* keyA = (uint32_t*)c.zkeys;
        uint32_t* keyB = keyA + cap_z;
        uint32_t* idxA = (uint32_t*)zkeys_b;
        uint32_t* idxB = idxA + cap_z;
        if ((int64_t)cap_z >= 4096 * (int64_t)Zs) k_zsort_layers<8><<<Zs, ZS_THREADS, 0, st>>>(c, keyA, keyB, idxA, idxB, zperm);
        else k_zsort_layers<1><<<Zs, ZS_THREADS, 0, st>>>(c, keyA, keyB, idxA, idxB, zperm);
        t3d_count_launches(1);
    }
    if (phases & 2) {
        if (t3d_zero_async(counts + 2, 8, st)) return 1;
        if (cap_g0 > 0) {
            k_gsort<<<1, ZS_THREADS, 0, st>>>(c, c.gkeys, gkeys_b, c.gval, (uint32_t*)temp, gperm);
        }
        k_canon_positions<<<(unsigned)((V + 255) / 256), 256, 0, st>>>(c);
        if (canonical_tail(c.verts, c.perm, V, (const unsigned long long*)V_dev_u64, faces_in, F, (const unsigned long long*)F_dev_u64,
                           verts_out, faces_out_i64, faces_out_i32, counts, flags, pos, newid, scan_ws, scan_ws_f, totals, st)) return 1;
        t3d_count_launches((F > 0 ? 5 : 3) + (cap_g0 > 0 ? 1 : 0));
    }
    T3D_CHECK_LAUNCH("t3d_mesh_canonicalize_structured");
    return 0;
}

template <typename IdxT>
__global__ void __launch_bounds__(256) k_mesh_measure(const float* __restrict__ verts, const IdxT* __restrict__ faces, int64_t F_cap,
                                                      double* __restrict__ partials, const unsigned long long* __restrict__ F_dev = nullptr)
{
    const int64_t F = dev_n(F_cap, F_dev);
    double vol = 0.0, area = 0.0;
    for (int64_t i = (int64_t)blockIdx.x * blockDim.x + threadIdx.x; i < F; i += (int64_t)gridDim.x * blockDim.x) {
        const float* a = verts + 3 * (int64_t)faces[3 * i];
        const float* b = verts + 3 * (int64_t)faces[3 * i + 1];
        const float* c = verts + 3 * (int64_t)faces[3 * i + 2];
        const double ax = a[0], ay = a[1], az = a[2], bx = b[0], by = b[1], bz = b[2], cx = c[0], cy = c[1], cz = c[2];
        const double nx = by * cz - bz * cy, ny = bz * cx - bx * cz, nz = bx * cy - by * cx;
        vol += (ax * nx + ay * ny + az * nz) / 6.0;
        const double ux = bx - ax, uy = by - ay, uz = bz - az, vx = cx - ax, vy = cy - ay, vz = cz - az;
        const double px = uy * vz - uz * vy, py = uz * vx - ux * vz, pz = ux * vy - uy * vx;
        area += 0.5 * sqrt(px * px + py * py + pz * pz);
    }
    vol = warp_sum(vol); area = warp_sum(area);
    __shared__ double sv[8], sa[8];
    if (lane_id() == 0) { sv[threadIdx.x >> 5] = vol; sa[threadIdx.x >> 5] = area; }
    __syncthreads();
    if (threadIdx.x == 0) {
        double v = 0, a = 0;
        for (int k = 0; k < 8; ++k) { v += sv[k]; a += sa[k]; }
        partials[2 * blockIdx.x] = v; partials[2 * blockIdx.x + 1] = a;
    }
}

__global__ void __launch_bounds__(256) k_reduce_partials(const double* __restrict__ partials, int n, double* __restrict__ out)
{
    double v = 0, a = 0;
    for (int i = threadIdx.x; i < n; i += 256) { v += partials[2 * i]; a += partials[2 * i + 1]; }
    v = warp_sum(v); a = warp_sum(a);
    __shared__ double sv[8], sa[8];
    if (lane_id() == 0) { sv[threadIdx.x >> 5] = v; sa[threadIdx.x >> 5] = a; }
    __syncthreads();
    if (threadIdx.x == 0) {
        double tv = 0, ta = 0;
        for (int k = 0; k < 8; ++k) { tv += sv[k]; ta += sa[k]; }
        out[0] = tv; out[1] = ta;
    }
}

#define MM_BLOCKS (T3D_NUM_SMS * 4)

extern "C" int64_t t3d_mesh_measure_workspace_bytes(void) { return (int64_t)MM_BLOCKS * 2 * 8; }

extern "C" int t3d_mesh_measure_dev(const void* verts_f32, const void* faces, int64_t F, const void* F_dev_u64, int faces_are_i64,
                                    void* out_f64, void* workspace, void* stream)
{
    cudaStream_t st = (cudaStream_t)stream;
    const unsigned long long* F_dev = (const unsigned long long*)F_dev_u64;
    if (F <= 0) { T3D_CUDA(cudaMemsetAsync(out_f64, 0, 16, st)); return 0; }
    int blocks = (int)((F + 255) / 256);
    if (blocks > MM_BLOCKS) blocks = MM_BLOCKS;
    if (faces_are_i64)
        k_mesh_measure<long long><<<blocks, 256, 0, st>>>((const float*)verts_f32, (const long long*)faces, F, (double*)workspace, F_dev);
    else
        k_mesh_measure<int32_t><<<blocks, 256, 0, st>>>((const float*)verts_f32, (const int32_t*)faces, F, (double*)workspace, F_dev);
    k_reduce_partials<<<1, 256, 0, st>>>((const double*)workspace, blocks, (double*)out_f64);
    T3D_CHECK_LAUNCH("t3d_mesh_measure_dev");
    t3d_count_launches(2);
    return 0;
}
```

Measured before the change: 857.4.

## Fuse mesh volume/area measurement into face remap and compact faces with lookback scan

```diff
diff --git a/tomography_3d_reconstructor_b200/csrc/t3d_common.cuh b/tomography_3d_reconstructor_b200/csrc/t3d_common.cuh
--- a/tomography_3d_reconstructor_b200/csrc/t3d_common.cuh
+++ b/tomography_3d_reconstructor_b200/csrc/t3d_common.cuh
@@ -136,6 +136,21 @@
                       unsigned long long* counts, cudaStream_t st);
 void t3d_canon_faces_ready_event(cudaEvent_t e);
 bool t3d_canon_faces_ready_pending();
+struct RawMeshMeasure {
+    const float* verts;
+    double* partials;
+    double* out;
+};
+int t3d_canonicalize_fast_measured(const void* verts_in, int64_t V, const void* V_dev_u64, const void* faces_in, int64_t F,
+                                   const void* F_dev_u64, void* verts_out, void* faces_out_i64, void* faces_out_i32, void* counts_u64,
+                                   void* workspace, const RawMeshMeasure* measure, void* stream);
+int t3d_canonicalize_structured_measured(const void* verts_in, const void* vkeys_u64, int64_t V_cap, const void* sizes_u64,
+                                         const void* V_dev_u64, int Zs, int Hs, int Ws, const void* chunkbase_u32, const void* aw_base_u32,
+                                         uint32_t aw_stride, int z_offset, int unpad_shift, const void* cum_f64, const void* adj_f64,
+                                         int n_cum, int zkey_bits, uint32_t cap_z, uint32_t cap_g0, const void* faces_in, int64_t F_cap,
+                                         const void* F_dev_u64, void* verts_out, void* faces_out_i64, void* faces_out_i32,
+                                         void* counts_u64, void* n_g0_u64, void* workspace, int phases, const RawMeshMeasure* measure,
+                                         void* stream);
 bool t3d_pack_gap_supported(const void* masks_u8, int Z, int H, int W, int threshold);
 int t3d_pack_gap_launch(const void* masks_u8, int Z, int H, int W, int threshold, void* out, unsigned long long* counts,
                         unsigned int* bbox_t, int skip_ends, cudaStream_t st, int z_bias = 0);
diff --git a/tomography_3d_reconstructor_b200/csrc/t3d_pipeline.cu b/tomography_3d_reconstructor_b200/csrc/t3d_pipeline.cu
--- a/tomography_3d_reconstructor_b200/csrc/t3d_pipeline.cu
+++ b/tomography_3d_reconstructor_b200/csrc/t3d_pipeline.cu
@@ -366,25 +366,22 @@
     RUN(t3d_mc_emit_view_dev(view, x_off, ws + L.sign, Zp, Hp, Wp, g.z_begin, g.z_end, ws + L.ballots, ws + L.chunkbase, ws + L.aw_idx,
                              ws + L.aw_base, cap_active, R + R_NACTIVE, cap_verts, cap_faces, ws + L.vkeys, ws + L.faces_raw, 2, side->s));
     T3D_CUDA(cudaEventRecord(side->e[6], side->s));
-    RUN(t3d_mesh_measure_dev(ws + L.verts_raw, ws + L.faces_raw, cap_faces, R + R_NT, 0, R + R_VOLUME_F64, ws + L.measure, side->s));
-    T3D_CUDA(cudaEventRecord(side->e[5], side->s));
     t3d_canon_faces_ready_event(side->e[6]);
+    const RawMeshMeasure measure = {(const float*)(ws + L.verts_raw), (double*)(ws + L.measure), (double*)(R + R_VOLUME_F64)};
     if (cap_zverts)
-        RUN(t3d_mesh_canonicalize_structured_dev(ws + L.verts_raw, ws + L.vkeys, cap_verts, R + R_NACTIVE, R + R_VRAW, Zp, Hp, Wp,
+        RUN(t3d_canonicalize_structured_measured(ws + L.verts_raw, ws + L.vkeys, cap_verts, R + R_NACTIVE, R + R_VRAW, Zp, Hp, Wp,
                                                  ws + L.chunkbase, ws + L.aw_base, cap_active, g.z_offset, 1, cum_f64, adj_f64, n_cum,
                                                  zkey_bits, cap_zverts, cap_g0, ws + L.faces_raw, cap_faces, R + R_NT, verts_out_f32,
-                                                 faces_out_i64, nullptr, R + R_VCANON, R + R_NG0, ws + L.canon, 3, st));
+                                                 faces_out_i64, nullptr, R + R_VCANON, R + R_NG0, ws + L.canon, 3, &measure, st));
     else
-        RUN(t3d_mesh_canonicalize_fast_dev(ws + L.verts_raw, cap_verts, R + R_VRAW, ws + L.faces_raw, cap_faces, R + R_NT,
-                                           verts_out_f32, faces_out_i64, nullptr, R + R_VCANON, ws + L.canon, st));
+        RUN(t3d_canonicalize_fast_measured(ws + L.verts_raw, cap_verts, R + R_VRAW, ws + L.faces_raw, cap_faces, R + R_NT,
+                                           verts_out_f32, faces_out_i64, nullptr, R + R_VCANON, ws + L.canon, &measure, st));
     if (t3d_canon_faces_ready_pending()) T3D_CUDA(cudaStreamWaitEvent(st, side->e[6], 0));
     if (g.want_ghost || g.want_lead)
         k_count_plane_vertices<<<1, 64, 0, st>>>((const float*)verts_out_f32, R + R_VCANON, g.z_ghost, g.z_lead, g.want_ghost,
                                                  g.want_lead, R + R_NGHOST, R + R_NLEAD);
     if (g.want_ghost || g.want_lead) t3d_count_launches(1);
     marks.mark("canonicalize", st);
-    T3D_CUDA(cudaStreamWaitEvent(st, side->e[5], 0));
-    marks.mark("wait measures", st);
     marks.report(st);
     return 0;
 }
diff --git a/tomography_3d_reconstructor_b200/csrc/t3d_surface.cu b/tomography_3d_reconstructor_b200/csrc/t3d_surface.cu
--- a/tomography_3d_reconstructor_b200/csrc/t3d_surface.cu
+++ b/tomography_3d_reconstructor_b200/csrc/t3d_surface.cu
@@ -131,6 +131,34 @@
 #define SC_FLAG_P (2ull << 62)
 #define SC_VALUE_MASK ((1ull << 62) - 1)
 
+__device__ __forceinline__ unsigned long long tile_lookback(volatile unsigned long long* d, int tile, unsigned long long agg)
+{
+    const int lane = threadIdx.x & 31;
+    if (tile == 0) {
+        if (lane == 0) d[0] = SC_FLAG_P | agg;
+        return 0;
+    }
+    if (lane == 0) d[tile] = SC_FLAG_A | agg;
+    unsigned long long prefix = 0;
+    int idx = tile - 1 - lane;
+    while (true) {
+        unsigned long long w = (idx >= 0) ? d[idx] : SC_FLAG_P;
+        while (__any_sync(0xffffffffu, (w >> 62) == 0)) {
+            if ((w >> 62) == 0) w = (idx >= 0) ? d[idx] : SC_FLAG_P;
+        }
+        const uint32_t is_p = __ballot_sync(0xffffffffu, (w >> 62) == 2);
+        const int first_p = is_p ? (__ffs(is_p) - 1) : 32;
+        unsigned long long val = (lane <= first_p) ? (w & SC_VALUE_MASK) : 0ull;
+#pragma unroll
+        for (int off = 16; off > 0; off >>= 1) val += __shfl_xor_sync(0xffffffffu, val, off);
+        prefix += val;
+        if (is_p) break;
+        idx -= 32;
+    }
+    if (lane == 0) d[tile] = SC_FLAG_P | ((prefix + agg) & SC_VALUE_MASK);
+    return prefix;
+}
+
 template <typename OutT>
 __global__ void __launch_bounds__(SC_THREADS) k_scan_lookback(const uint32_t* __restrict__ in, OutT* __restrict__ out, int64_t n_cap,
                                                               int64_t stride, unsigned long long* __restrict__ desc, int n_tiles,
@@ -169,28 +197,7 @@
         agg += sh[k];
     }
     if (threadIdx.x < 32) {
-        unsigned long long prefix = 0;
-        if (tile == 0) {
-            if (threadIdx.x == 0) { d[0] = SC_FLAG_P | (unsigned long long)agg; }
-        } else {
-            if (threadIdx.x == 0) { d[tile] = SC_FLAG_A | (unsigned long long)agg; }
-            int idx = tile - 1 - (int)threadIdx.x;
-            while (true) {
-                unsigned long long w = (idx >= 0) ? d[idx] : SC_FLAG_P;
-                while (__any_sync(0xffffffffu, (w >> 62) == 0)) {
-                    if ((w >> 62) == 0) w = (idx >= 0) ? d[idx] : SC_FLAG_P;
-                }
-                const uint32_t is_p = __ballot_sync(0xffffffffu, (w >> 62) == 2);
-                const int first_p = is_p ? (__ffs(is_p) - 1) : 32;
-                unsigned long long val = ((int)threadIdx.x <= first_p) ? (w & SC_VALUE_MASK) : 0ull;
-#pragma unroll
-                for (int off = 16; off > 0; off >>= 1) val += __shfl_xor_sync(0xffffffffu, val, off);
-                prefix += val;
-                if (is_p) break;
-                idx -= 32;
-            }
-            if (threadIdx.x == 0) { d[tile] = SC_FLAG_P | ((prefix + agg) & SC_VALUE_MASK); }
-        }
+        const unsigned long long prefix = tile_lookback(d, tile, agg);
         if (threadIdx.x == 0) {
             s_prefix = prefix;
             if (tile == n_tiles - 1) totals[blockIdx.y] = prefix + agg;
@@ -398,30 +405,163 @@
     }
 }
 
-__global__ void __launch_bounds__(256) k_face_remap(const int32_t* __restrict__ faces, int64_t F_cap, const uint32_t* __restrict__ newid,
+#define MM_BLOCKS (T3D_NUM_SMS * 4)
+
+struct FaceVerts {
+    float a[3], b[3], c[3];
+};
+
+__device__ __forceinline__ FaceVerts load_face_verts(const float* __restrict__ verts, int64_t ia, int64_t ib, int64_t ic)
+{
+    FaceVerts f;
+#pragma unroll
+    for (int k = 0; k < 3; ++k) { f.a[k] = verts[3 * ia + k]; f.b[k] = verts[3 * ib + k]; f.c[k] = verts[3 * ic + k]; }
+    return f;
+}
+
+__device__ __forceinline__ void face_measure_terms(const FaceVerts& f, double& vol, double& area)
+{
+    const double ax = f.a[0], ay = f.a[1], az = f.a[2], bx = f.b[0], by = f.b[1], bz = f.b[2], cx = f.c[0], cy = f.c[1], cz = f.c[2];
+    const double nx = __fma_rn(by, cz, -__dmul_rn(bz, cy)), ny = __fma_rn(bz, cx, -__dmul_rn(bx, cz)),
+                 nz = __fma_rn(bx, cy, -__dmul_rn(by, cx));
+    vol = __dadd_rn(vol, __ddiv_rn(__fma_rn(az, nz, __fma_rn(ax, nx, __dmul_rn(ay, ny))), 6.0));
+    const double ux = __dsub_rn(bx, ax), uy = __dsub_rn(by, ay), uz = __dsub_rn(bz, az);
+    const double vx = __dsub_rn(cx, ax), vy = __dsub_rn(cy, ay), vz = __dsub_rn(cz, az);
+    const double px = __fma_rn(uy, vz, -__dmul_rn(uz, vy)), py = __fma_rn(uz, vx, -__dmul_rn(ux, vz)),
+                 pz = __fma_rn(ux, vy, -__dmul_rn(uy, vx));
+    area = __fma_rn(__dsqrt_rn(__fma_rn(pz, pz, __fma_rn(px, px, __dmul_rn(py, py)))), 0.5, area);
+}
+
+__device__ __forceinline__ void measure_block_partial(double vol, double area, double* __restrict__ partials)
+{
+    vol = warp_sum(vol); area = warp_sum(area);
+    __shared__ double sv[8], sa[8];
+    if (lane_id() == 0) { sv[threadIdx.x >> 5] = vol; sa[threadIdx.x >> 5] = area; }
+    __syncthreads();
+    if (threadIdx.x == 0) {
+        double v = 0, a = 0;
+        for (int k = 0; k < 8; ++k) { v += sv[k]; a += sa[k]; }
+        partials[2 * blockIdx.x] = v; partials[2 * blockIdx.x + 1] = a;
+    }
+}
+
+__device__ __forceinline__ void measure_reduce_partials(const double* partials, int n, double* __restrict__ out)
+{
+    double v = 0, a = 0;
+    for (int i = threadIdx.x; i < n; i += 256) { v += __ldcg(partials + 2 * i); a += __ldcg(partials + 2 * i + 1); }
+    v = warp_sum(v); a = warp_sum(a);
+    __shared__ double sv[8], sa[8];
+    if (lane_id() == 0) { sv[threadIdx.x >> 5] = v; sa[threadIdx.x >> 5] = a; }
+    __syncthreads();
+    if (threadIdx.x == 0) {
+        double tv = 0, ta = 0;
+        for (int k = 0; k < 8; ++k) { tv += sv[k]; ta += sa[k]; }
+        out[0] = tv; out[1] = ta;
+    }
+}
+
+__device__ __forceinline__ bool remap_face(int64_t i, uint32_t a, uint32_t b, uint32_t c,
+                                           uint32_t* __restrict__ valid, long long* __restrict__ out64, int32_t* __restrict__ out32)
+{
+    const bool ok = a != b && b != c && a != c;
+    valid[i] = ok ? 1u : 0u;
+    if (out64) { out64[3 * i] = a; out64[3 * i + 1] = b; out64[3 * i + 2] = c; }
+    if (out32) { out32[3 * i] = (int32_t)a; out32[3 * i + 1] = (int32_t)b; out32[3 * i + 2] = (int32_t)c; }
+    return ok;
+}
+
+__global__ void __launch_bounds__(256, 4) k_face_remap(const int32_t* __restrict__ faces, int64_t F_cap, const uint32_t* __restrict__ newid,
                                                     uint32_t* __restrict__ valid, long long* __restrict__ out64, int32_t* __restrict__ out32,
-                                                    unsigned long long* __restrict__ n_invalid, const unsigned long long* __restrict__ F_dev)
-{
-    const int64_t i = (int64_t)blockIdx.x * blockDim.x + threadIdx.x;
+                                                    const float* __restrict__ verts, double* partials, double* __restrict__ measures,
+                                                    unsigned long long* n_invalid, unsigned int* __restrict__ ticket,
+                                                    unsigned long long* __restrict__ f_out, const unsigned long long* __restrict__ F_dev)
+{
     const int64_t F = dev_n(F_cap, F_dev);
-    bool bad = false;
+    double vol = 0.0, area = 0.0;
+    uint32_t bad = 0;
+    const int64_t stride = (int64_t)gridDim.x * blockDim.x;
+    int64_t i = (int64_t)blockIdx.x * blockDim.x + threadIdx.x;
+    for (; i + stride < F; i += 2 * stride) {
+        const int64_t j = i + stride;
+        const int32_t ra = faces[3 * i], rb = faces[3 * i + 1], rc = faces[3 * i + 2];
+        const int32_t sa = faces[3 * j], sb = faces[3 * j + 1], sc = faces[3 * j + 2];
+        const uint32_t a = newid[ra], b = newid[rb], c = newid[rc], a2 = newid[sa], b2 = newid[sb], c2 = newid[sc];
+        FaceVerts f0, f1;
+        if (verts) { f0 = load_face_verts(verts, ra, rb, rc); f1 = load_face_verts(verts, sa, sb, sc); }
+        bad += remap_face(i, a, b, c, valid, out64, out32) ? 0u : 1u;
+        bad += remap_face(j, a2, b2, c2, valid, out64, out32) ? 0u : 1u;
+        if (verts) { face_measure_terms(f0, vol, area); face_measure_terms(f1, vol, area); }
+    }
     if (i < F) {
-        const uint32_t a = newid[faces[3 * i]], b = newid[faces[3 * i + 1]], c = newid[faces[3 * i + 2]];
-        bad = !(a != b && b != c && a != c);
-        valid[i] = bad ? 0u : 1u;
-        if (out64) { out64[3 * i] = a; out64[3 * i + 1] = b; out64[3 * i + 2] = c; }
-        if (out32) { out32[3 * i] = (int32_t)a; out32[3 * i + 1] = (int32_t)b; out32[3 * i + 2] = (int32_t)c; }
-    }
-    const uint32_t nb = __popc(__ballot_sync(0xffffffffu, bad));
-    if (lane_id() == 0 && nb) atomicAdd(n_invalid, (unsigned long long)nb);
-}
-
-__global__ void k_face_plan(const unsigned long long* __restrict__ n_invalid, int64_t F_cap, const unsigned long long* __restrict__ F_dev,
-                            unsigned long long* __restrict__ n_to_compact, unsigned long long* __restrict__ f_out)
-{
-    const unsigned long long F = (unsigned long long)dev_n(F_cap, F_dev);
-    *n_to_compact = (*n_invalid) ? F : 0ull;
-    *f_out = F - *n_invalid;
+        const int32_t ra = faces[3 * i], rb = faces[3 * i + 1], rc = faces[3 * i + 2];
+        bad += remap_face(i, newid[ra], newid[rb], newid[rc], valid, out64, out32) ? 0u : 1u;
+        if (verts) face_measure_terms(load_face_verts(verts, ra, rb, rc), vol, area);
+    }
+    bad = warp_sum(bad);
+    if (lane_id() == 0 && bad) atomicAdd(n_invalid, (unsigned long long)bad);
+    if (verts) measure_block_partial(vol, area, partials);
+    __shared__ bool s_last;
+    __threadfence();
+    __syncthreads();
+    if (threadIdx.x == 0) s_last = atomicAdd(ticket, 1u) == gridDim.x - 1;
+    __syncthreads();
+    if (!s_last) return;
+    if (threadIdx.x == 0) *f_out = (unsigned long long)F - atomicAdd(n_invalid, 0ull);
+    if (verts) measure_reduce_partials(partials, (int)gridDim.x, measures);
+}
+
+__global__ void __launch_bounds__(SC_THREADS) k_face_compact_lookback(const int32_t* __restrict__ faces, int64_t F_cap,
+                                                                      const uint32_t* __restrict__ newid, const uint32_t* __restrict__ valid,
+                                                                      long long* __restrict__ out64, int32_t* __restrict__ out32,
+                                                                      unsigned long long* __restrict__ desc, int n_tiles,
+                                                                      unsigned int* __restrict__ ticket,
+                                                                      const unsigned long long* __restrict__ n_invalid,
+                                                                      const unsigned long long* __restrict__ F_dev)
+{
+    if (*n_invalid == 0) return;
+    const int64_t n = dev_n(F_cap, F_dev);
+    __shared__ int s_tile;
+    __shared__ uint32_t sh[SC_THREADS / 32];
+    __shared__ unsigned long long s_prefix;
+    if (threadIdx.x == 0) s_tile = (int)atomicAdd(ticket, 1u);
+    __syncthreads();
+    const int tile = s_tile;
+    const int64_t need = (n + SC_TILE - 1) / SC_TILE;
+    n_tiles = (int)(need < 1 ? 1 : (need < n_tiles ? need : n_tiles));
+    if (tile >= n_tiles) return;
+    const int64_t base = (int64_t)tile * SC_TILE + (int64_t)threadIdx.x * SC_ITEMS;
+    uint32_t v[SC_ITEMS];
+    uint32_t sum = 0;
+#pragma unroll
+    for (int k = 0; k < SC_ITEMS; ++k) {
+        v[k] = (base + k < n) ? valid[base + k] : 0u;
+        sum += v[k];
+    }
+    const uint32_t incl = warp_incl_scan(sum);
+    if (lane_id() == 31) sh[threadIdx.x >> 5] = incl;
+    __syncthreads();
+    uint32_t woff = 0, agg = 0;
+#pragma unroll
+    for (int k = 0; k < SC_THREADS / 32; ++k) {
+        if (k < (int)(threadIdx.x >> 5)) woff += sh[k];
+        agg += sh[k];
+    }
+    if (threadIdx.x < 32) {
+        const unsigned long long prefix = tile_lookback(desc, tile, agg);
+        if (threadIdx.x == 0) s_prefix = prefix;
+    }
+    __syncthreads();
+    int64_t run = (int64_t)s_prefix + woff + (incl - sum);
+#pragma unroll
+    for (int k = 0; k < SC_ITEMS; ++k) {
+        const int64_t i = base + k;
+        if (i < n && v[k]) {
+            const uint32_t a = newid[faces[3 * i]], b = newid[faces[3 * i + 1]], c = newid[faces[3 * i + 2]];
+            if (out64) { out64[3 * run] = a; out64[3 * run + 1] = b; out64[3 * run + 2] = c; }
+            if (out32) { out32[3 * run] = (int32_t)a; out32[3 * run + 1] = (int32_t)b; out32[3 * run + 2] = (int32_t)c; }
+        }
+        run += v[k];
+    }
 }
 
 static size_t sort_temp_bytes(int64_t V)
@@ -543,7 +683,7 @@
     int64_t b = 0;
     b += 2 * align256(8 * V);
     b += 2 * align256(4 * V);
-    b += 2 * align256(4 * n);
+    b += align256(4 * n);
     b += align256(4 * V);
     b += align256((int64_t)sort64_temp_bytes(V > 0 ? V : 1));
     b += align256(t3d_scan_workspace_bytes(n, 1));
@@ -624,28 +764,7 @@
         uint32_t runp = incl - psum;
 #pragma unroll
         for (int t = 0; t < PER_LANE; ++t) { s_part[PER_LANE * lane + t] = runp; runp += pv[t]; }
-        unsigned long long prefix = 0;
-        if (tile == 0) {
-            if (tid == 0) { d[0] = SC_FLAG_P | (unsigned long long)agg; }
-        } else {
-            if (tid == 0) { d[tile] = SC_FLAG_A | (unsigned long long)agg; }
-            int idx = tile - 1 - tid;
-            while (true) {
-                unsigned long long w = (idx >= 0) ? d[idx] : SC_FLAG_P;
-                while (__any_sync(0xffffffffu, (w >> 62) == 0)) {
-                    if ((w >> 62) == 0) w = (idx >= 0) ? d[idx] : SC_FLAG_P;
-                }
-                const uint32_t is_p = __ballot_sync(0xffffffffu, (w >> 62) == 2);
-                const int first_p = is_p ? (__ffs(is_p) - 1) : 32;
-                unsigned long long val = (tid <= first_p) ? (w & SC_VALUE_MASK) : 0ull;
-#pragma unroll
-                for (int off = 16; off > 0; off >>= 1) val += __shfl_xor_sync(0xffffffffu, val, off);
-                prefix += val;
-                if (is_p) break;
-                idx -= 32;
-            }
-            if (tid == 0) { d[tile] = SC_FLAG_P | ((prefix + agg) & SC_VALUE_MASK); }
-        }
+        const unsigned long long prefix = tile_lookback(d, tile, agg);
         if (tid == 0) {
             s_prefix = prefix;
             if (tile == n_tiles - 1) *n_unique_out = prefix + agg;
@@ -705,10 +824,9 @@
 
 static int canonical_tail(const float* vin, const uint32_t* perm, int64_t V, const unsigned long long* V_dev, const void* faces_in,
                           int64_t F, const unsigned long long* F_dev, void* verts_out, void* faces_out_i64, void* faces_out_i32,
-                          unsigned long long* counts, uint32_t* flags, uint32_t* pos, uint32_t* newid, void* scan_ws,
-                          void* scan_ws_faces, unsigned long long* totals, cudaStream_t st)
-{
-    void* stream = (void*)st;
+                          unsigned long long* counts, uint32_t* flags, uint32_t* newid, void* scan_ws, void* scan_ws_faces,
+                          unsigned long long* totals, const RawMeshMeasure* measure, cudaStream_t st)
+{
     {
         const int64_t nb = (V + UQ_TILE - 1) / UQ_TILE;
         const size_t desc_bytes = (size_t)nb * 8;
@@ -725,15 +843,17 @@
         g_faces_ready = nullptr;
     }
     if (F > 0) {
-        const unsigned gf = (unsigned)((F + 255) / 256);
-        if (t3d_zero_async(totals + 1, 16, st)) return 1;
-        k_face_remap<<<gf, 256, 0, st>>>((const int32_t*)faces_in, F, newid, flags, (long long*)faces_out_i64, (int32_t*)faces_out_i32,
-                                         totals + 1, F_dev);
-        k_face_plan<<<1, 1, 0, st>>>(totals + 1, F, F_dev, totals + 2, counts + 1);
-        if (t3d_exclusive_scan_u32_dev(flags, pos, F, F, 1, 0, 0, totals + 2, totals + 3, scan_ws_faces, stream)) return 1;
-        const unsigned gc = gf < (unsigned)(T3D_NUM_SMS * 8) ? gf : (unsigned)(T3D_NUM_SMS * 8);
-        k_face_compact<<<gc, 256, 0, st>>>((const int32_t*)faces_in, F, newid, flags, pos, (long long*)faces_out_i64,
-                                           (int32_t*)faces_out_i32, totals + 2);
+        const int64_t gf = (F + 255) / 256;
+        const unsigned gm = (unsigned)(gf < MM_BLOCKS ? gf : MM_BLOCKS);
+        const int64_t nt = (F + SC_TILE - 1) / SC_TILE;
+        const size_t desc_bytes = (size_t)nt * 8;
+        if (t3d_zero_async(totals + 1, 16, st) || t3d_zero_async(scan_ws_faces, desc_bytes + 64, st)) return 1;
+        k_face_remap<<<gm, 256, 0, st>>>((const int32_t*)faces_in, F, newid, flags, (long long*)faces_out_i64, (int32_t*)faces_out_i32,
+                                         measure ? measure->verts : nullptr, measure ? measure->partials : nullptr,
+                                         measure ? measure->out : nullptr, totals + 1, (unsigned int*)(totals + 2), counts + 1, F_dev);
+        k_face_compact_lookback<<<(unsigned)nt, SC_THREADS, 0, st>>>((const int32_t*)faces_in, F, newid, flags, (long long*)faces_out_i64,
+                                                                    (int32_t*)faces_out_i32, (unsigned long long*)scan_ws_faces, (int)nt,
+                                                                    (unsigned int*)((char*)scan_ws_faces + desc_bytes), totals + 1, F_dev);
     } else {
         T3D_CUDA(cudaMemsetAsync(counts + 1, 0, 8, st));
     }
@@ -743,6 +863,14 @@
 extern "C" int t3d_mesh_canonicalize_fast_dev(const void* verts_in, int64_t V, const void* V_dev_u64, const void* faces_in, int64_t F,
                                               const void* F_dev_u64, void* verts_out, void* faces_out_i64, void* faces_out_i32,
                                               void* counts_u64, void* workspace, void* stream)
+{
+    return t3d_canonicalize_fast_measured(verts_in, V, V_dev_u64, faces_in, F, F_dev_u64, verts_out, faces_out_i64, faces_out_i32,
+                                          counts_u64, workspace, nullptr, stream);
+}
+
+int t3d_canonicalize_fast_measured(const void* verts_in, int64_t V, const void* V_dev_u64, const void* faces_in, int64_t F,
+                                   const void* F_dev_u64, void* verts_out, void* faces_out_i64, void* faces_out_i32, void* counts_u64,
+                                   void* workspace, const RawMeshMeasure* measure, void* stream)
 {
     cudaStream_t st = (cudaStream_t)stream;
     if (V <= 0 || V > 0x7fffffff || F < 0) { t3d_set_error("t3d_mesh_canonicalize_fast_dev: bad sizes"); return 2; }
@@ -755,7 +883,6 @@
     uint32_t* iota = (uint32_t*)ws; ws += align256(4 * V);
     uint32_t* perm = (uint32_t*)ws; ws += align256(4 * V);
     uint32_t* flags = (uint32_t*)ws; ws += align256(4 * n);
-    uint32_t* pos = (uint32_t*)ws; ws += align256(4 * n);
     uint32_t* newid = (uint32_t*)ws; ws += align256(4 * V);
     size_t temp_bytes = sort64_temp_bytes(V);
     void* temp = ws; ws += align256((int64_t)temp_bytes);
@@ -768,10 +895,10 @@
     k_make_keys64<<<gv, 256, 0, st>>>(vin, V, V_dev, keys_a, iota);
     T3D_CUDA(cub::DeviceRadixSort::SortPairs(temp, temp_bytes, (const unsigned long long*)keys_a, keys_b, (const uint32_t*)iota, perm,
                                              (int)V, 0, 64, st));
-    if (canonical_tail(vin, perm, V, V_dev, faces_in, F, F_dev, verts_out, faces_out_i64, faces_out_i32, counts, flags, pos, newid,
-                       scan_ws, scan_ws, totals, st)) return 1;
+    if (canonical_tail(vin, perm, V, V_dev, faces_in, F, F_dev, verts_out, faces_out_i64, faces_out_i32, counts, flags, newid,
+                       scan_ws, scan_ws, totals, measure, st)) return 1;
     T3D_CHECK_LAUNCH("t3d_mesh_canonicalize_fast_dev");
-    t3d_count_launches(F > 0 ? 5 : 3);
+    t3d_count_launches(F > 0 ? 4 : 3);
     return 0;
 }
 
@@ -859,6 +986,7 @@
     __shared__ uint32_t s_hist[ZS_WARPS][256];
     __shared__ uint32_t s_tot[256];
     __shared__ uint32_t s_carry[8];
+    __shared__ KeyT s_kmax;
     const int tid = threadIdx.x, w = tid >> 5, lane = tid & 31;
     const uint32_t per = (((n + ZS_WARPS - 1) / ZS_WARPS) + 31u) & ~31u;
     const uint32_t ws = min(n, (uint32_t)w * per), we = min(n, ws + per);
@@ -866,21 +994,32 @@
     KeyT* kout = keyB; uint32_t* iout = idxB;
     for (int p = 0; p < passes; ++p) {
         const int shift = 8 * p;
-        const bool first = p == 0, last = p == passes - 1;
+        const bool first = p == 0;
         for (int i = tid; i < ZS_WARPS * 256; i += ZS_THREADS) (&s_hist[0][0])[i] = 0;
+        if (first && tid == 0) s_kmax = 0;
         __syncthreads();
+        KeyT kmax = 0;
         for (uint32_t i0 = ws + lane; i0 < we; i0 += 32 * ZS_U) {
             KeyT kk[ZS_U];
 #pragma unroll
             for (int u = 0; u < ZS_U; ++u) {
                 const uint32_t i = i0 + 32 * u;
-                if (i < we) { if (first) { kk[u] = key_of(i); keyA[i] = kk[u]; } else kk[u] = kin[i]; }
+                if (i < we) {
+                    if (first) { kk[u] = key_of(i); keyA[i] = kk[u]; kmax = kk[u] > kmax ? kk[u] : kmax; }
+                    else kk[u] = kin[i];
+                }
             }
 #pragma unroll
             for (int u = 0; u < ZS_U; ++u)
                 if (i0 + 32 * u < we) atomicAdd(&s_hist[w][(uint32_t)(kk[u] >> shift) & 255u], 1u);
         }
+        if (kmax) atomicMax(&s_kmax, kmax);
         __syncthreads();
+        if (first) {
+            const int bits = sizeof(KeyT) == 8 ? 64 - __clzll((long long)s_kmax) : 32 - __clz((int)s_kmax);
+            passes = min(passes, max(1, (bits + 7) / 8));
+        }
+        const bool last = p == passes - 1;
         if (tid < 256) {
             uint32_t t = 0;
             for (int ww = 0; ww < ZS_WARPS; ++ww) t += s_hist[ww][tid];
@@ -1027,7 +1166,7 @@
     b += 2 * align256(8 * (int64_t)cap_z) + 2 * align256(4 * (int64_t)cap_z);
     b += 2 * align256(8 * (int64_t)cap_g0) + 2 * align256(4 * (int64_t)cap_g0);
     b += align256(4 * V);
-    b += 2 * align256(4 * n);
+    b += align256(4 * n);
     b += align256(4 * V);
     b += align256(4 * (int64_t)cap_g0 + 256);
     b += 2 * align256(t3d_scan_workspace_bytes(n, 1)) + 256;
@@ -1050,7 +1189,7 @@
     if (kind == 1) {
         o = 2 * align256(8 * V) + align256(4 * V);
         out4[1] = o; o += align256(4 * V);
-        out4[2] = o; o += 2 * align256(4 * n);
+        out4[2] = o; o += align256(4 * n);
         out4[0] = o; o += align256(4 * V);
         o += align256((int64_t)sort64_temp_bytes(V));
         o += align256(t3d_scan_workspace_bytes(n, 1));
@@ -1058,7 +1197,7 @@
         o = 2 * align256(8 * (int64_t)cap_z) + 2 * align256(4 * (int64_t)cap_z) + 2 * align256(8 * (int64_t)cap_g0) +
             2 * align256(4 * (int64_t)cap_g0);
         out4[1] = o; o += align256(4 * V);
-        out4[2] = o; o += 2 * align256(4 * n);
+        out4[2] = o; o += align256(4 * n);
         out4[0] = o; o += align256(4 * V);
         o += align256(4 * (int64_t)cap_g0 + 256);
         o += 2 * align256(t3d_scan_workspace_bytes(n, 1));
@@ -1083,6 +1222,20 @@
                                                     uint32_t cap_z, uint32_t cap_g0, const void* faces_in, int64_t F_cap,
                                                     const void* F_dev_u64, void* verts_out, void* faces_out_i64, void* faces_out_i32,
                                                     void* counts_u64, void* n_g0_u64, void* workspace, int phases, void* stream)
+{
+    return t3d_canonicalize_structured_measured(verts_in, vkeys_u64, V_cap, sizes_u64, V_dev_u64, Zs, Hs, Ws, chunkbase_u32, aw_base_u32,
+                                                aw_stride, z_offset, unpad_shift, cum_f64, adj_f64, n_cum, zkey_bits, cap_z, cap_g0,
+                                                faces_in, F_cap, F_dev_u64, verts_out, faces_out_i64, faces_out_i32, counts_u64, n_g0_u64,
+                                                workspace, phases, nullptr, stream);
+}
+
+int t3d_canonicalize_structured_measured(const void* verts_in, const void* vkeys_u64, int64_t V_cap, const void* sizes_u64,
+                                         const void* V_dev_u64, int Zs, int Hs, int Ws, const void* chunkbase_u32, const void* aw_base_u32,
+                                         uint32_t aw_stride, int z_offset, int unpad_shift, const void* cum_f64, const void* adj_f64,
+                                         int n_cum, int zkey_bits, uint32_t cap_z, uint32_t cap_g0, const void* faces_in, int64_t F_cap,
+                                         const void* F_dev_u64, void* verts_out, void* faces_out_i64, void* faces_out_i32,
+                                         void* counts_u64, void* n_g0_u64, void* workspace, int phases, const RawMeshMeasure* measure,
+                                         void* stream)
 {
     cudaStream_t st = (cudaStream_t)stream;
     if (zkey_bits <= 0 || zkey_bits > 32) zkey_bits = 32;
@@ -1117,7 +1270,6 @@
     gperm = (uint32_t*)ws; ws += align256(4 * (int64_t)cap_g0);
     c.perm = (uint32_t*)ws; ws += align256(4 * V);
     uint32_t* flags = (uint32_t*)ws; ws += align256(4 * n);
-    uint32_t* pos = (uint32_t*)ws; ws += align256(4 * n);
     uint32_t* newid = (uint32_t*)ws; ws += align256(4 * V);
     void* temp = ws; ws += align256(4 * (int64_t)cap_g0 + 256);
     void* scan_ws = ws; ws += align256(t3d_scan_workspace_bytes(n, 1));
@@ -1142,8 +1294,8 @@
         }
         k_canon_positions<<<(unsigned)((V + 255) / 256), 256, 0, st>>>(c);
         if (canonical_tail(c.verts, c.perm, V, (const unsigned long long*)V_dev_u64, faces_in, F, (const unsigned long long*)F_dev_u64,
-                           verts_out, faces_out_i64, faces_out_i32, counts, flags, pos, newid, scan_ws, scan_ws_f, totals, st)) return 1;
-        t3d_count_launches((F > 0 ? 5 : 3) + (cap_g0 > 0 ? 1 : 0));
+                           verts_out, faces_out_i64, faces_out_i32, counts, flags, newid, scan_ws, scan_ws_f, totals, measure, st)) return 1;
+        t3d_count_launches((F > 0 ? 4 : 3) + (cap_g0 > 0 ? 1 : 0));
     }
     T3D_CHECK_LAUNCH("t3d_mesh_canonicalize_structured");
     return 0;
@@ -1155,44 +1307,15 @@
 {
     const int64_t F = dev_n(F_cap, F_dev);
     double vol = 0.0, area = 0.0;
-    for (int64_t i = (int64_t)blockIdx.x * blockDim.x + threadIdx.x; i < F; i += (int64_t)gridDim.x * blockDim.x) {
-        const float* a = verts + 3 * (int64_t)faces[3 * i];
-        const float* b = verts + 3 * (int64_t)faces[3 * i + 1];
-        const float* c = verts + 3 * (int64_t)faces[3 * i + 2];
-        const double ax = a[0], ay = a[1], az = a[2], bx = b[0], by = b[1], bz = b[2], cx = c[0], cy = c[1], cz = c[2];
-        const double nx = by * cz - bz * cy, ny = bz * cx - bx * cz, nz = bx * cy - by * cx;
-        vol += (ax * nx + ay * ny + az * nz) / 6.0;
-        const double ux = bx - ax, uy = by - ay, uz = bz - az, vx = cx - ax, vy = cy - ay, vz = cz - az;
-        const double px = uy * vz - uz * vy, py = uz * vx - ux * vz, pz = ux * vy - uy * vx;
-        area += 0.5 * sqrt(px * px + py * py + pz * pz);
-    }
-    vol = warp_sum(vol); area = warp_sum(area);
-    __shared__ double sv[8], sa[8];
-    if (lane_id() == 0) { sv[threadIdx.x >> 5] = vol; sa[threadIdx.x >> 5] = area; }
-    __syncthreads();
-    if (threadIdx.x == 0) {
-        double v = 0, a = 0;
-        for (int k = 0; k < 8; ++k) { v += sv[k]; a += sa[k]; }
-        partials[2 * blockIdx.x] = v; partials[2 * blockIdx.x + 1] = a;
-    }
+    for (int64_t i = (int64_t)blockIdx.x * blockDim.x + threadIdx.x; i < F; i += (int64_t)gridDim.x * blockDim.x)
+        face_measure_terms(load_face_verts(verts, (int64_t)faces[3 * i], (int64_t)faces[3 * i + 1], (int64_t)faces[3 * i + 2]), vol, area);
+    measure_block_partial(vol, area, partials);
 }
 
 __global__ void __launch_bounds__(256) k_reduce_partials(const double* __restrict__ partials, int n, double* __restrict__ out)
 {
-    double v = 0, a = 0;
-    for (int i = threadIdx.x; i < n; i += 256) { v += partials[2 * i]; a += partials[2 * i + 1]; }
-    v = warp_sum(v); a = warp_sum(a);
-    __shared__ double sv[8], sa[8];
-    if (lane_id() == 0) { sv[threadIdx.x >> 5] = v; sa[threadIdx.x >> 5] = a; }
-    __syncthreads();
-    if (threadIdx.x == 0) {
-        double tv = 0, ta = 0;
-        for (int k = 0; k < 8; ++k) { tv += sv[k]; ta += sa[k]; }
-        out[0] = tv; out[1] = ta;
-    }
-}
-
-#define MM_BLOCKS (T3D_NUM_SMS * 4)
+    measure_reduce_partials(partials, n, out);
+}
 
 extern "C" int64_t t3d_mesh_measure_workspace_bytes(void) { return (int64_t)MM_BLOCKS * 2 * 8; }
 
```

New measurement: 876.0 (median of 6 runs). 2.2% higher.
